# Illumina/canvas

Measured on AMD Instinct MI355X. Metric: genome-bins/sec (bin+clean+partition), higher is better.
Workload: dtype u8/int32 (bin), f32/f64 (clean, viterbi); 1 GPU; BASELINE configs[2]: whole-genome GRCh38 60x single sample, full bin+clean+partition HIP path on 1 MI355X per sample; bins_after_clean=4686240, bin_size=534, partition=PerSampleHMM, clean_flags=-g -s -r --local-sd-metric-file, segments=250, samples=1

## Files before the change

canvas_amd/csrc/hmm.hip:

```cpp
#include "common.hpp"
#include <type_traits>
#include "select.hpp"
#include "quantize.hpp"
#include <mutex>
#include <cmath>
#include <thread>
#include <cstring>
#include <limits>
#include <algorithm>

#define NSTATE 5

struct HmmParams {
    double logA[NSTATE][NSTATE];
    double logPi[NSTATE];
    int32_t tableLen;
    double maxThreshold;
};

__global__ void __launch_bounds__(256) k_keys_cov_f32(const double* __restrict__ cov, int64_t n, uint32_t* __restrict__ keys) {
    int64_t i = (int64_t)blockIdx.x * 256 + threadIdx.x;
    if (i < n) keys[i] = key_of_float((float)cov[i]);
}

// ... 260 lines not shown
struct __attribute__((aligned(2))) VecH8 { uint32_t w[4]; };

template <int J, bool TWO = false>
__device__ __forceinline__ void vit_state(const double (&d)[NSTATE], double e, const HmmParams& P, double& outDelta, uint32_t& outArg) {
    const double NEG = -1.7976931348623157e308;
    const double cOff = e + P.logA[J == 0 ? 1 : 0][J], cDiag = e + P.logA[J][J];
    const double t_0 = d[0] + (TWO ? (J == 0 ? cDiag : cOff) : (e + P.logA[0][J]));
    const double t_1 = d[1] + (TWO ? (J == 1 ? cDiag : cOff) : (e + P.logA[1][J]));
    const double t_2 = d[2] + (TWO ? (J == 2 ? cDiag : cOff) : (e + P.logA[2][J]));
    const double t_3 = d[3] + (TWO ? (J == 3 ? cDiag : cOff) : (e + P.logA[3][J]));
    const double t_4 = d[4] + (TWO ? (J == 4 ? cDiag : cOff) : (e + P.logA[4][J]));
    double a = __builtin_fmax(__builtin_fmax(__builtin_fmax(t_0, t_1), __builtin_fmax(t_2, t_3)), t_4);
    uint32_t ia = t_3 == a ? 3u : 4u;
    ia = t_2 == a ? 2u : ia; ia = t_1 == a ? 1u : ia; ia = t_0 == a ? 0u : ia;
    if (!(a > NEG)) { a = NEG; ia = 0; }
    outDelta = a; outArg = ia;
}
template <bool TWO = false>
__device__ __forceinline__ uint32_t vit_step5(double (&d)[NSTATE], const double (&e)[NSTATE], const HmmParams& P) {
    double n0, n1, n2, n3, n4; uint32_t a0, a1, a2, a3, a4;
    vit_state<0, TWO>(d, e[0], P, n0, a0); vit_state<1, TWO>(d, e[1], P, n1, a1); vit_state<2, TWO>(d, e[2], P, n2, a2);
    vit_state<3, TWO>(d, e[3], P, n3, a3); vit_state<4, TWO>(d, e[4], P, n4, a4);
    d[0] = n0; d[1] = n1; d[2] = n2; d[3] = n3; d[4] = n4;
    return a0 | (a1 << 3) | (a2 << 6) | (a3 << 9) | (a4 << 12);
}
__device__ __forceinline__ void vit_init5(double (&d)[NSTATE], const double (&e)[NSTATE], const HmmParams& P) {
#pragma unroll
    for (int j = 0; j < NSTATE; j++) { double lik = e[j] + P.logA[0][j]; d[j] = P.logPi[j] + lik - P.logA[0][j]; }
}
__device__ __forceinline__ int vit_best5(const double (&d)[NSTATE]) {
    int best = -1; double m1 = -1.7976931348623157e308;
#pragma unroll
    for (int i = 0; i < NSTATE; i++) if (d[i] > m1) { best = i; m1 = d[i]; }
    return best;
}
__device__ __forceinline__ uint32_t map_get(uint32_t m, uint32_t j) { return (m >> (3u * j)) & 7u; }
__device__ __forceinline__ uint32_t map_compose(uint32_t outer, uint32_t inner) {
    return map_get(outer, map_get(inner, 0)) | (map_get(outer, map_get(inner, 1)) << 3) | (map_get(outer, map_get(inner, 2)) << 6) |
           (map_get(outer, map_get(inner, 3)) << 9) | (map_get(outer, map_get(inner, 4)) << 12);
}
__device__ __forceinline__ double sel5(const double (&d)[NSTATE], uint32_t i) {
    double r = d[0];
    r = i == 1 ? d[1] : r; r = i == 2 ? d[2] : r; r = i == 3 ? d[3] : r; r = i == 4 ? d[4] : r;
    return r;
}
__device__ __forceinline__ void vit_emissions(double (&e)[NSTATE], const double* __restrict__ sTab, const double* __restrict__ logPmf, bool useLds, int tableLen, int k) {
    if (useLds) {
#pragma unroll
        for (int j = 0; j < NSTATE; j++) e[j] = sTab[k * NSTATE + j];
    } else {
#pragma unroll
        for (int j = 0; j < NSTATE; j++) e[j] = logPmf[(size_t)j * tableLen + k];
    }
}
__device__ __forceinline__ void vit_stage_table(double* sTab, const double* __restrict__ logPmf, int tableLen, bool useLds) {
    if (useLds) for (int i = threadIdx.x; i < tableLen * NSTATE; i += blockDim.x) { int s = i / tableLen, k = i - s * tableLen; sTab[k * NSTATE + s] = logPmf[i]; }
    __syncthreads();
}
__device__ __forceinline__ int wave_max_i32(int v) {
#pragma unroll
    for (int d = 32; d >= 1; d >>= 1) { int o = __shfl_xor(v, d); v = o > v ? o : v; }
    return v;
}

template <typename T> __device__ __forceinline__ void make_block_entry(const int32_t* __restrict__ first, int nchr, int i, int per, T* __restrict__ out) {
    int lo = 0, hi = nchr - 1;
    while (lo < hi) { int mid = (lo + hi + 1) >> 1; if (first[mid] <= i) lo = mid; else hi = mid - 1; }
    while (lo < nchr - 1 && first[lo + 1] <= i) lo++;
    T b; b.chrom = lo; b.t0 = (i - first[lo]) * per;
    out[i] = b;
}
template <typename T>
__global__ void __launch_bounds__(256) k_make_blocks(const int32_t* __restrict__ first, int nchr, int n, int per, T* __restrict__ out) {
    const int i = blockIdx.x * 256 + threadIdx.x;
    if (i < n) make_block_entry(first, nchr, i, per, out);
}

#define HMM_BYVAL 64
struct HmmDescPack { HmmChrom chroms[HMM_BYVAL]; int64_t off[HMM_BYVAL + 1]; int32_t first[HMM_BYVAL + 1], firstChunk[HMM_BYVAL + 1], firstS[HMM_BYVAL + 1], firstGroup[HMM_BYVAL + 1]; };
struct HmmDescDev { HmmChrom* chroms; int64_t* off; int32_t* first; int32_t* firstChunk; int32_t* firstS; int32_t* firstGroup; };
template <typename VB_T, typename BB_T>
__global__ void __launch_bounds__(256) k_hmm_setup(const HmmDescPack pack, int usePack, HmmDescDev D, int nchr,
                                                   int nblocks, int nblocksS, int nchunks, int vb, int vbs, int bbChunk, VB_T* __restrict__ vBlocks, VB_T* __restrict__ sBlocks, BB_T* __restrict__ bChunks,
                                                   const double* __restrict__ cov, int64_t N, double maxThreshold, int32_t* __restrict__ idx, int32_t* __restrict__ dLast, int32_t* __restrict__ dFail) {
    const int32_t* first = usePack ? pack.first : D.first; const int32_t* firstS = usePack ? pack.firstS : D.firstS; const int32_t* firstChunk = usePack ? pack.firstChunk : D.firstChunk;
    if (usePack && blockIdx.x == 0) {
        for (int c = threadIdx.x; c < nchr; c += 256) D.chroms[c] = pack.chroms[c];
        for (int c = threadIdx.x; c <= nchr; c += 256) { D.off[c] = pack.off[c]; D.first[c] = pack.first[c]; D.firstChunk[c] = pack.firstChunk[c]; D.firstS[c] = pack.firstS[c]; D.firstGroup[c] = pack.firstGroup[c]; }
    }
    const int64_t i = (int64_t)blockIdx.x * 256 + threadIdx.x;
    if (i < nblocks) make_block_entry(first, nchr, (int)i, vb, vBlocks);
    if (i < nblocksS) make_block_entry(firstS, nchr, (int)i, vbs, sBlocks);
    if (i < nchunks) make_block_entry(firstChunk, nchr, (int)i, bbChunk, bChunks);
    if (i < nchr) { dLast[i] = -1; dFail[i] = 0; }
    if (cov && i < N) {
        double x = cov[i];
        x = x > maxThreshold ? maxThreshold : x;
        const int32_t k = (int32_t)rint(x);
        idx[i] = k < 0 ? 0 : k;
    }
}

template <bool useLds, bool TWO>
__global__ void __launch_bounds__(64) k_vit_spec(const VitBlock* __restrict__ blocks, int nblocks, const HmmChrom* __restrict__ chroms, const int32_t* __restrict__ idx,
                                                 const double* __restrict__ logPmf, HmmParams P, uint16_t* __restrict__ psi, uint16_t* __restrict__ maps,
                                                 int32_t* __restrict__ lastGuess, int leadIn, const int32_t* __restrict__ todo, int vb) {
    extern __shared__ double sTab[];
    vit_stage_table(sTab, logPmf, P.tableLen, useLds);
    const int b = blockIdx.x * 64 + threadIdx.x;
    const bool actBlock = b < nblocks;
    const VitBlock B = blocks[actBlock ? b : nblocks - 1];
    const HmmChrom C = chroms[B.chrom];
    const int64_t tBeg = B.t0, tEnd = (B.t0 + vb < C.T) ? B.t0 + vb : C.T;
    const int64_t ts = tBeg > leadIn ? tBeg - leadIn : 0;
    const bool act = actBlock && (!todo || todo[B.chrom]);
    const int nsteps = act ? (int)(tEnd - ts) : 0;
    const int maxSteps = wave_max_i32(nsteps);
    const int32_t* __restrict__ ix = idx + C.begin + ts;
    uint16_t* __restrict__ pp = psi + C.begin;
    double d[NSTATE] = {0.0, 0.0, 0.0, 0.0, 0.0};
    uint32_t fm = MAP_IDENT;
    const int lead = (int)(tBeg - ts);
    if (nsteps > 0) {
        double e[NSTATE];
        vit_emissions(e, sTab, logPmf, useLds, P.tableLen, ix[0]);
        if (ts == 0) vit_init5(d, e, P);
        else {
#pragma unroll
            for (int j = 0; j < NSTATE; j++) d[j] = e[j];
        }
        if (lead == 0) pp[ts] = 0;
    }
    VecI4 qa = *reinterpret_cast<const VecI4*>(ix + 1), qb = *reinterpret_cast<const VecI4*>(ix + 5);
    double eCur[NSTATE];
    vit_emissions(eCur, sTab, logPmf, useLds, P.tableLen, 1 < nsteps ? qa.v[0] : 0);
    auto group = [&](int s0, auto withMaps) {
        constexpr bool WM = decltype(withMaps)::value;
        const VecI4 na = *reinterpret_cast<const VecI4*>(ix + s0 + PQ), nb = *reinterpret_cast<const VecI4*>(ix + s0 + PQ + 4);
        uint32_t pks[PQ];
#pragma unroll
        for (int u = 0; u < PQ; u++) {
            const int s = s0 + u;
            const bool on = s < nsteps;
            const int kNext = (s + 1 < nsteps) ? (u + 1 < 4 ? qa.v[(u + 1) & 3] : (u + 1 < 8 ? qb.v[(u + 1) & 3] : na.v[0])) : 0;
            double eNext[NSTATE], dn[NSTATE];
            vit_emissions(eNext, sTab, logPmf, useLds, P.tableLen, kNext);
#pragma unroll
            for (int j = 0; j < NSTATE; j++) dn[j] = d[j];
            const uint32_t pk = vit_step5<TWO>(dn, eCur, P);
#pragma unroll
            for (int j = 0; j < NSTATE; j++) { d[j] = on ? dn[j] : d[j]; eCur[j] = eNext[j]; }
            if (WM) { fm = (on && s >= lead) ? map_compose(fm, pk) : fm; pks[u] = pk; }
        }
        if (WM) {
#pragma unroll
            for (int u = 0; u < PQ; u++) { const int s = s0 + u; if (s < nsteps && s >= lead) pp[ts + s] = (uint16_t)pks[u]; }
        }
        qa = na; qb = nb;
    };
    const int leadMin = -wave_max_i32(nsteps > 0 ? -lead : -0x7FFFFFFF);
    int s0 = 1;
    for (; s0 + PQ <= leadMin && s0 < maxSteps; s0 += PQ) group(s0, std::false_type{});
    for (; s0 < maxSteps; s0 += PQ) group(s0, std::true_type{});
    if (act) {
        maps[b] = (uint16_t)fm;
        if (tEnd == C.T) lastGuess[B.chrom] = vit_best5(d);
    }
}

#define CHR_LDS_CAP 1024
__device__ __forceinline__ const int64_t* stage_chr_offsets(const int64_t* __restrict__ chrOff, int nchr, int64_t* sOff) {
    if (nchr + 1 > CHR_LDS_CAP) return chrOff;
    for (int k = threadIdx.x; k <= nchr; k += blockDim.x) sOff[k] = chrOff[k];
    __syncthreads();
    return sOff;
}
__device__ __forceinline__ int chrom_of_bin(const int64_t* off, int nchr, int64_t g) {
    int lo = 0, hi = nchr - 1;
    while (lo < hi) { const int mid = (lo + hi + 1) >> 1; if (off[mid] <= g) lo = mid; else hi = mid - 1; }
    return lo;
}
#define VBS (VB / 2)
__global__ void __launch_bounds__(256) k_pair_maps(const VitBlock* __restrict__ blocks, int nblocks, const HmmChrom* __restrict__ chroms, const int32_t* __restrict__ firstS,
                                                   const uint16_t* __restrict__ mapsS, uint16_t* __restrict__ maps, const int32_t* __restrict__ todo) {
    const int b = blockIdx.x * 256 + threadIdx.x;
    if (b >= nblocks) return;
    const VitBlock B = blocks[b];
    if (todo && !todo[B.chrom]) return;
    const int64_t T = chroms[B.chrom].T;
    const int s0 = firstS[B.chrom] + B.t0 / VBS;
    uint32_t m = mapsS[s0];
#pragma unroll
    for (int k = 1; k < VB / VBS; k++) if (B.t0 + (int64_t)k * VBS < T) m = map_compose(m, mapsS[s0 + k]);
    maps[b] = (uint16_t)m;
}

__global__ void __launch_bounds__(256) k_vit_increments(const HmmChrom* __restrict__ chroms, int nchr, const int64_t* __restrict__ chrOff, const int32_t* __restrict__ idx,
                                                        const double* __restrict__ logPmf, HmmParams P, const int32_t* __restrict__ state, int64_t N, double* __restrict__ D) {
    __shared__ int64_t sOff[CHR_LDS_CAP];
    const int64_t* off = stage_chr_offsets(chrOff, nchr, sOff);
    int64_t g = (int64_t)blockIdx.x * 256 + threadIdx.x;
    if (g >= N) return;
    const int s1 = state[g], sPrev = state[g > 0 ? g - 1 : 0], ix = idx[g];
    const int lo = chrom_of_bin(off, nchr, g);
    const int64_t begin = chroms[lo].begin;
    if (s1 < 0) { D[g] = 0.0; return; }
    double e = logPmf[(size_t)s1 * P.tableLen + ix];
    if (g == begin) { double lik = e + P.logA[0][s1]; D[g] = P.logPi[s1] + lik - P.logA[0][s1]; }
    else { const int s0 = sPrev; D[g] = e + P.logA[s0 < 0 ? 0 : s0][s1]; }
}

__global__ void __launch_bounds__(64) k_vit_backbone(const HmmChrom* __restrict__ chroms, const double* __restrict__ V, double* __restrict__ carryOut, const int32_t* __restrict__ todo = nullptr) {
    __shared__ double sV[2][64];
    const HmmChrom C = chroms[blockIdx.x];
    if (C.T <= 10 || (todo && !todo[blockIdx.x])) return;
    const int l = threadIdx.x;
    const double* __restrict__ Vc = V + C.begin;
    double acc = 0.0;
    double vNext = l < C.T ? Vc[l] : 0.0;
    int buf = 0;
    for (int64_t c0 = 0; c0 < C.T; c0 += 64, buf ^= 1) {
        sV[buf][l] = vNext;
        { int64_t t2 = c0 + 64 + l; vNext = t2 < C.T ? Vc[t2] : 0.0; }
        if (l == 0) carryOut[C.begin + c0] = acc;
        double r[64];
#pragma unroll
        for (int s = 0; s < 64; s++) r[s] = sV[buf][s];
#pragma unroll
        for (int s = 0; s < 64; s++) acc = acc + r[s];
    }
}

#define BS_T 1024
#define BS_I 8
struct ParFn { unsigned long long a0, a1; };
__device__ __forceinline__ ParFn parfn_then(ParFn f, ParFn g) {
    ParFn h;
    h.a0 = f.a0 + ((f.a0 & 1ull) ? g.a1 : g.a0);
    h.a1 = f.a1 + ((f.a1 & 1ull) ? g.a0 : g.a1);
    return h;
}
__device__ __forceinline__ ParFn parfn_shfl_up(ParFn f, int d) {
    ParFn o;
    o.a0 = __shfl_up(f.a0, d); o.a1 = __shfl_up(f.a1, d);
    return o;
}
__global__ void __launch_bounds__(BS_T) k_vit_backbone_scan(const HmmChrom* __restrict__ chroms, const double* __restrict__ V, double* __restrict__ carryOut, int32_t* __restrict__ fail) {
    __shared__ ParFn sAgg[BS_T / 64];
    __shared__ long long sCross, sP;
    __shared__ double sM;
    __shared__ int sBad;
    const HmmChrom C = chroms[blockIdx.x];
    if (C.T <= 10) return;
    const int tid = threadIdx.x, lane = tid & 63, wave = tid >> 6;
    const double* __restrict__ Vc = V + C.begin;
    double* __restrict__ carry = carryOut + C.begin;
    const unsigned long long TWO53 = 1ull << 53, MANT = (1ull << 52) - 1ull;
    if (tid == 0) { carry[0] = 0.0; sM = 0.0; sP = 0; sBad = 0; sCross = 0x7fffffffffffffffll; }
    __syncthreads();
    for (;;) {
        const long long p = sP; const double M = sM; const int bad = sBad;
        __syncthreads();
        if (bad || p >= C.T) break;
        if (!(M >= 2.2250738585072014e-308)) {
            if (tid == 0) {
                const double v = Vc[p];
                const unsigned long long vb = (unsigned long long)__double_as_longlong(v);
                if (((vb >> 52) & 0x7ffull) == 0x7ffull || (!(vb >> 63) && (vb << 1) != 0ull)) { sBad = 1; fail[blockIdx.x] = 1; }
                else { const double acc = (0.0 - M) + v; if (((p + 1) & 63) == 0 && p + 1 < C.T) carry[p + 1] = acc; sM = -acc; sP = p + 1; }
            }
            __syncthreads();
            continue;
        }
        const unsigned long long mb = (unsigned long long)__double_as_longlong(M);
        const int eM = (int)((mb >> 52) & 0x7ffull);
        const unsigned long long k0 = (mb & MANT) | (1ull << 52);
        const long long base = p + (long long)tid * BS_I;
        ParFn f[BS_I]; bool myBad = false;
#pragma unroll
        for (int i = 0; i < BS_I; i++) {
            const long long t = base + i;
            unsigned long long A = 0; int r = 0;
            if (t < C.T) {
                const unsigned long long vb = (unsigned long long)__double_as_longlong(Vc[t]);
                const int ea = (int)((vb >> 52) & 0x7ffull);
                if (ea == 0x7ff || (!(vb >> 63) && (vb << 1) != 0ull)) myBad = true;
                const unsigned long long ma = ea ? ((vb & MANT) | (1ull << 52)) : (vb & MANT);
                const int shift = eM - (ea ? ea : 1);
                if (shift <= 0) { if (ma) A = TWO53; }
                else if (shift < 64) {
                    A = ma >> shift;
                    const unsigned long long rem = ma & ((1ull << shift) - 1ull), half = 1ull << (shift - 1);
// ... 118 lines not shown
    const BbChunk K = chunks[blockIdx.x];
    const HmmChrom C = chroms[K.chrom];
    const double* __restrict__ Vc = V + C.begin;
    const int tid = threadIdx.x, lane = tid & 63, wave = tid >> 6;
    unsigned long long vb[4]; double a[4]; bool in[4];
#pragma unroll
    for (int i = 0; i < 4; i++) {
        const int64_t t = (int64_t)K.t0 + tid * 4 + i;
        in[i] = t < C.T;
        const double v = in[i] ? Vc[t] : 0.0;
        vb[i] = (unsigned long long)__double_as_longlong(v); a[i] = fabs(v);
    }
    const double tsum = ((a[0] + a[1]) + a[2]) + a[3];
    double inc = tsum;
#pragma unroll
    for (int d = 1; d < 64; d <<= 1) { double o = shfl_up_f64(inc, d); if (lane >= d) inc += o; }
    if (lane == 63) swSum[wave] = inc;
    __syncthreads();
    double base = chunkBase[blockIdx.x];
    for (int w = 0; w < wave; w++) base += swSum[w];
    double Mprev = base + (inc - tsum);
    SegFn el[4];
#pragma unroll
    for (int i = 0; i < 4; i++) {
        const double Mcur = Mprev + a[i];
        const int ep = (int)(((unsigned long long)__double_as_longlong(Mprev) >> 52) & 0x7ffull), ec = (int)(((unsigned long long)__double_as_longlong(Mcur) >> 52) & 0x7ffull);
        const bool cross = in[i] && (ep == 0 || ec != ep);
        el[i].head = cross ? 1u : 0u; el[i].cnt = cross ? 1u : 0u;
        if (cross || !in[i]) { el[i].f.a0 = 0; el[i].f.a1 = 0; }
        else el[i].f = parfn_of(vb[i], ep);
        a[i] = Mcur;
        Mprev = Mcur;
    }
    SegFn th = el[0];
#pragma unroll
    for (int i = 1; i < 4; i++) th = segfn_then(th, el[i]);
    SegFn sc = th;
#pragma unroll
    for (int d = 1; d < 64; d <<= 1) {
        SegFn o; o.f = parfn_shfl_up(sc.f, d); o.head = __shfl_up(sc.head, d); o.cnt = __shfl_up(sc.cnt, d);
        if (lane >= d) sc = segfn_then(o, sc);
    }
    if (lane == 63) swSeg[wave] = sc;
    __syncthreads();
    SegFn ex; ex.f.a0 = 0; ex.f.a1 = 0; ex.head = 0; ex.cnt = 0;
    for (int w = 0; w < wave; w++) ex = segfn_then(ex, swSeg[w]);
    { SegFn o; o.f = parfn_shfl_up(sc.f, 1); o.head = __shfl_up(sc.head, 1); o.cnt = __shfl_up(sc.cnt, 1); if (lane > 0) ex = segfn_then(ex, o); }
    SegFn run = ex;
    BbCross* __restrict__ myCross = outCross + (size_t)blockIdx.x * BB_MAXC;
    bool overflow = false;
#pragma unroll
    for (int i = 0; i < 4; i++) {
        const int pos = tid * 4 + i;
        if (el[i].head) {
            if (run.cnt < BB_MAXC) {
                BbCross R; R.before = run.f; R.v = __longlong_as_double((long long)vb[i]);
                R.pos = pos; R.e = (int)(((unsigned long long)__double_as_longlong(a[i]) >> 52) & 0x7ffull);
                myCross[run.cnt] = R;
            } else overflow = true;
        }
        run = segfn_then(run, el[i]);
        if ((pos & 63) == 63) {
            at64Fn[(size_t)blockIdx.x * 16 + (pos >> 6)] = run.f;
            at64Rank[(size_t)blockIdx.x * 16 + (pos >> 6)] = (uint8_t)((run.cnt > 127u ? 127u : run.cnt) | (el[i].head ? 0x80u : 0u));
        }
    }
    if (overflow) fail[K.chrom] = 1;
    if (tid == 0) {
        outChunk[blockIdx.x].headE = (int)(((unsigned long long)__double_as_longlong(base) >> 52) & 0x7ffull);
    }
    if (tid == 255) { outChunk[blockIdx.x].tail = run.f; outChunk[blockIdx.x].nCross = (int32_t)run.cnt; }
}
__device__ __forceinline__ bool bb_apply(unsigned long long& bits, const ParFn& f, int eUsed) {
    const unsigned long long MANT = (1ull << 52) - 1ull;
    if (f.a0 == 0ull && f.a1 == 0ull) return true;
    const int e = (int)(bits >> 52);
    if (e != eUsed || e == 0) return false;
    const unsigned long long k = (bits & MANT) | (1ull << 52);
    const unsigned long long k2 = k + ((k & 1ull) ? f.a1 : f.a0);
    if (k2 >= (1ull << 53)) return false;
    bits = ((unsigned long long)e << 52) | (k2 & MANT);
    return true;
}
__global__ void __launch_bounds__(64) k_bb_walk(const int32_t* __restrict__ firstChunk, const BbChunkOut* __restrict__ chunkOut, const BbCross* __restrict__ cross,
                                                unsigned long long* __restrict__ chunkBits, BbPost* __restrict__ post, int32_t* __restrict__ fail) {
    __shared__ BbCross sCr[BB_MAXC];
    const int c = blockIdx.x, l = threadIdx.x;
    const unsigned long long MANT = (1ull << 52) - 1ull;
    if (fail[c]) return;
    unsigned long long bits = 0ull;
    bool failed = false;
    for (int g = firstChunk[c]; g < firstChunk[c + 1] && !failed; g += 64) {
        const int n = firstChunk[c + 1] - g < 64 ? firstChunk[c + 1] - g : 64;
        BbChunkOut my; my.tail.a0 = 0; my.tail.a1 = 0; my.nCross = 0; my.headE = 0;
        if (l < n) my = chunkOut[g + l];
        unsigned long long crossMask = __ballot(l < n && my.nCross > 0);
        int cur = 0;
        while (cur < n && !failed) {
            const int f = crossMask ? (int)__builtin_ctzll(crossMask) : n;
            if (f > cur) {
                const bool inRun = l >= cur && l < f;
                ParFn inc; inc.a0 = inRun ? my.tail.a0 : 0ull; inc.a1 = inRun ? my.tail.a1 : 0ull;
#pragma unroll
                for (int d = 1; d < 64; d <<= 1) { ParFn o = parfn_shfl_up(inc, d); if (l >= d) inc = parfn_then(o, inc); }
                ParFn ex = parfn_shfl_up(inc, 1); if (l == 0) { ex.a0 = 0; ex.a1 = 0; }
                const int e = (int)(bits >> 52);
                const unsigned long long k = (bits & MANT) | (e ? (1ull << 52) : 0ull);
                const unsigned long long ks = k + ((k & 1ull) ? ex.a1 : ex.a0), ke = k + ((k & 1ull) ? inc.a1 : inc.a0);
                const bool nonEmpty = my.tail.a0 != 0ull || my.tail.a1 != 0ull;
                const bool bad = inRun && nonEmpty && (my.headE != e || e == 0 || ke >= (1ull << 53));
                if (inRun) chunkBits[g + l] = ((unsigned long long)e << 52) | (ks & MANT);
                if (__ballot(bad)) failed = true;
                const unsigned long long totLo0 = __shfl(inc.a0, f - 1), totLo1 = __shfl(inc.a1, f - 1);
                const unsigned long long k2 = k + ((k & 1ull) ? totLo1 : totLo0);
                bits = ((unsigned long long)e << 52) | (k2 & MANT);
                cur = f;
            }
            if (cur < n && !failed) {
                const int nc = __shfl(my.nCross, cur), headE = __shfl(my.headE, cur);
                ParFn tail; tail.a0 = __shfl(my.tail.a0, cur); tail.a1 = __shfl(my.tail.a1, cur);
                if (l < nc && l < BB_MAXC) sCr[l] = cross[(size_t)(g + cur) * BB_MAXC + l];
                __builtin_amdgcn_fence(__ATOMIC_ACQ_REL, "wavefront"); __builtin_amdgcn_wave_barrier();
                if (l == 0) chunkBits[g + cur] = bits;
                int eCur = headE;
                for (int r = 0; r < nc && r < BB_MAXC && !failed; r++) {
                    const BbCross R = sCr[r];
                    if (!bb_apply(bits, R.before, eCur)) { failed = true; break; }
                    const double acc = -__longlong_as_double((long long)bits) + R.v;
                    bits = (unsigned long long)__double_as_longlong(-acc) & ~(1ull << 63);
                    if ((int)(bits >> 52) != R.e) failed = true;
                    if (l == 0) post[(size_t)(g + cur) * BB_MAXC + r].bits = bits;
                    eCur = R.e;
                }
                if (!failed && !bb_apply(bits, tail, eCur)) failed = true;
                __builtin_amdgcn_fence(__ATOMIC_ACQ_REL, "wavefront"); __builtin_amdgcn_wave_barrier();
                crossMask &= ~(1ull << cur);
                cur++;
            }
        }
    }
    if (failed && l == 0) fail[c] = 1;
}
__global__ void __launch_bounds__(256) k_bb_emit(const BbChunk* __restrict__ chunks, int nchunks, const HmmChrom* __restrict__ chroms, const unsigned long long* __restrict__ chunkBits,
                                                 const BbPost* __restrict__ post, const ParFn* __restrict__ at64Fn, const uint8_t* __restrict__ at64Rank, double* __restrict__ carryOut) {
    const int i = blockIdx.x * 256 + threadIdx.x;
    const int c = i >> 4, q = i & 15;
    if (c >= nchunks) return;
    const BbChunk K = chunks[c];
    const HmmChrom C = chroms[K.chrom];
    if (q == 0 && K.t0 == 0) carryOut[C.begin] = 0.0;
    const int64_t t = (int64_t)K.t0 + q * 64 + 63;
    if (t + 1 >= C.T) return;
    const unsigned long long MANT = (1ull << 52) - 1ull;
    const uint32_t rk = at64Rank[i];
    const uint32_t rank = (rk & 0x7fu) > (uint32_t)BB_MAXC ? (uint32_t)BB_MAXC : (rk & 0x7fu);
    unsigned long long bits = rank == 0 ? chunkBits[c] : post[(size_t)c * BB_MAXC + (rank - 1)].bits;
    if (!(rk & 0x80u)) {
        const ParFn f = at64Fn[i];
        if (f.a0 != 0ull || f.a1 != 0ull) {
            const unsigned long long k = (bits & MANT) | (1ull << 52);
            const unsigned long long k2 = k + ((k & 1ull) ? f.a1 : f.a0);
            bits = (bits & ~MANT) | (k2 & MANT);
        }
    }
    carryOut[C.begin + t + 1] = -__longlong_as_double((long long)bits);
}

struct LogA25 { double a00, a01, a02, a03, a04, a10, a11, a12, a13, a14, a20, a21, a22, a23, a24, a30, a31, a32, a33, a34, a40, a41, a42, a43, a44; };
// ... 67 lines not shown
            for (int u = 0; u < PQ; u++) { const bool in = j0 + PQ + u < cnt; kn[u] = in ? ixp[j0 + PQ + u] : 0; sn[u] = in ? stp[j0 + PQ + u] : 0; vn[u] = in ? vp[j0 + PQ + u] : 0.0; }
#pragma unroll
            for (int u = 0; u < 4; u++) pn.w[u] = (uint32_t)(j0 + PQ + 2 * u < cnt ? ppp[j0 + PQ + 2 * u] : (uint16_t)0) | ((uint32_t)(j0 + PQ + 2 * u + 1 < cnt ? ppp[j0 + PQ + 2 * u + 1] : (uint16_t)0) << 16);
        }
#pragma unroll
        for (int u = 0; u < PQ; u++) {
            if (LEAD) ver_lead_step<useLds>(S, A, sTab, logPmf, P.tableLen, j0 + u < cnt, kq[u], sq[u], vq[u], pq[u]);
            else ver_block_step<useLds>(S, P, sTab, logPmf, j0 + u < cnt, kq[u], sq[u], vq[u], pq[u]);
        }
        __builtin_amdgcn_sched_barrier(0);
#pragma unroll
        for (int u = 0; u < PQ; u++) { kq[u] = kn[u]; sq[u] = sn[u]; vq[u] = vn[u]; pq[u] = (pn.w[u >> 1] >> (16 * (u & 1))) & 0xFFFFu; }
    }
}
template <bool useLds>
__global__ void __launch_bounds__(64) k_vit_verify(const VitBlock* __restrict__ blocks, int nblocks, const HmmChrom* __restrict__ chroms, const int32_t* __restrict__ idx,
                                                   const double* __restrict__ logPmf, HmmParams P, const uint16_t* __restrict__ psi,
                                                   const int32_t* __restrict__ state, const double* __restrict__ V, const double* __restrict__ carry, const int32_t* __restrict__ lastGuess,
                                                   int32_t* __restrict__ fail, int leadIn, const int32_t* __restrict__ todo) {
    extern __shared__ double sTab[];
    vit_stage_table(sTab, logPmf, P.tableLen, useLds);
    const int b = blockIdx.x * 64 + threadIdx.x;
    const bool actBlock = b < nblocks;
    const VitBlock B = blocks[actBlock ? b : nblocks - 1];
    const HmmChrom C = chroms[B.chrom];
    const int64_t tBeg = B.t0, tEnd = (B.t0 + VB < C.T) ? B.t0 + VB : C.T;
    const int64_t ts = tBeg > leadIn ? tBeg - leadIn : 0;
    const bool act = actBlock && (!todo || todo[B.chrom]);
    const int nsteps = act ? (int)(tEnd - ts) : 0;
    const int maxSteps = wave_max_i32(nsteps);
    const int32_t* __restrict__ ix = idx + C.begin + ts;
    const int32_t* __restrict__ st = state + C.begin + ts;
    const double* __restrict__ Vc = V + C.begin + ts;
    const uint16_t* __restrict__ pp = psi + C.begin + ts;
    VerState S;
#pragma unroll
    for (int j = 0; j < NSTATE; j++) S.d[j] = 0.0;
    S.valid = 0; S.bad = false; S.why = 0;
    S.Dprev = carry[C.begin + ts];
    S.sPrev = ts > 0 ? state[C.begin + ts - 1] : -1;
    LogA25 A;
#define LOGA_LOAD(i, j) A.a##i##j = P.logA[i][j]; asm volatile("" : "+v"(A.a##i##j));
    LOGA_LOAD(0, 0) LOGA_LOAD(0, 1) LOGA_LOAD(0, 2) LOGA_LOAD(0, 3) LOGA_LOAD(0, 4) LOGA_LOAD(1, 0) LOGA_LOAD(1, 1) LOGA_LOAD(1, 2) LOGA_LOAD(1, 3) LOGA_LOAD(1, 4)
    LOGA_LOAD(2, 0) LOGA_LOAD(2, 1) LOGA_LOAD(2, 2) LOGA_LOAD(2, 3) LOGA_LOAD(2, 4) LOGA_LOAD(3, 0) LOGA_LOAD(3, 1) LOGA_LOAD(3, 2) LOGA_LOAD(3, 3) LOGA_LOAD(3, 4)
    LOGA_LOAD(4, 0) LOGA_LOAD(4, 1) LOGA_LOAD(4, 2) LOGA_LOAD(4, 3) LOGA_LOAD(4, 4)
#undef LOGA_LOAD
    const int lead = (int)(tBeg - ts);
    if (nsteps > 0) {
        if (ts == 0) {
            double e[NSTATE];
            vit_emissions(e, sTab, logPmf, useLds, P.tableLen, ix[0]);
            const double Dt = S.Dprev + Vc[0];
            const int sCur = st[0];
            vit_init5(S.d, e, P); S.valid = 31u;
            if (sel5(S.d, (uint32_t)sCur) != Dt) { S.bad = true; S.why |= 16u; }
            S.Dprev = Dt; S.sPrev = sCur;
        } else ver_lead_step<useLds>(S, A, sTab, logPmf, P.tableLen, true, ix[0], st[0], Vc[0], (uint32_t)pp[0]);
    }
    const int start2 = lead > 1 ? lead : 1;
    ver_phase<useLds, true>(S, A, P, sTab, logPmf, ix + 1, st + 1, Vc + 1, pp + 1, nsteps > 0 && lead > 1 ? lead - 1 : 0);
    ver_phase<useLds, false>(S, A, P, sTab, logPmf, ix + start2, st + start2, Vc + start2, pp + start2, nsteps > start2 ? nsteps - start2 : 0);
    double (&d)[NSTATE] = S.d; const uint32_t valid = S.valid; bool bad = S.bad;
    uint32_t why = S.why;
    if (act && tEnd == C.T) { if (valid != 31u || vit_best5(d) != lastGuess[B.chrom]) { bad = true; why |= 32u; } }
    if (act && bad) atomicOr(&fail[B.chrom], (int32_t)(1u | why));
}

__global__ void k_vit_corrupt(uint16_t* __restrict__ psi, int64_t at, int j) {
    if (threadIdx.x == 0 && blockIdx.x == 0) { const uint32_t sh = 3u * (uint32_t)j; uint32_t v = psi[at], p = (v >> sh) & 7u; psi[at] = (uint16_t)((v & ~(7u << sh)) | (((p + 1u) % 5u) << sh)); }
}

__global__ void __launch_bounds__(256) k_bt_maps(const VitBlock* __restrict__ blocks, int nblocks, const HmmChrom* __restrict__ chroms, const uint16_t* __restrict__ psi,
                                                 uint16_t* __restrict__ maps) {
    int b = blockIdx.x * 256 + threadIdx.x;
    if (b >= nblocks) return;
    const VitBlock B = blocks[b];
    const HmmChrom C = chroms[B.chrom];
    const int64_t tBeg = B.t0 > 0 ? B.t0 : 1, tEnd = (B.t0 + VB < C.T) ? B.t0 + VB : C.T;
    uint32_t m = MAP_IDENT;
    for (int64_t t = tEnd - 1; t >= tBeg; t--) m = map_compose(psi[C.begin + t], m);
    maps[b] = (uint16_t)m;
}
__global__ void __launch_bounds__(64) k_bt_group(const int32_t* __restrict__ firstBlock, const int32_t* __restrict__ firstGroup, int nchr, const uint16_t* __restrict__ maps,
                                                 uint16_t* __restrict__ pre, uint16_t* __restrict__ gmap) {
    const int g = blockIdx.x, l = threadIdx.x;
    int lo = 0, hi = nchr - 1;
    while (lo < hi) { const int mid = (lo + hi + 1) >> 1; if (firstGroup[mid] <= g) lo = mid; else hi = mid - 1; }
    while (lo < nchr - 1 && firstGroup[lo + 1] <= g) lo++;
    const int first = firstBlock[lo], last = firstBlock[lo + 1] - 1;
    const int bi = last - ((g - firstGroup[lo]) * 64 + l);
    uint32_t f = bi >= first ? (uint32_t)maps[bi] : MAP_IDENT;
#pragma unroll
    for (int dlt = 1; dlt < 64; dlt <<= 1) { const uint32_t o = __shfl_up(f, dlt); if (l >= dlt) f = map_compose(f, o); }
    const uint32_t ex = __shfl_up(f, 1);
    if (bi >= first) pre[bi] = (uint16_t)(l == 0 ? MAP_IDENT : ex);
    if (l == 63) gmap[g] = (uint16_t)f;
}
__global__ void __launch_bounds__(64) k_bt_gchain(const int32_t* __restrict__ firstGroup, const int32_t* __restrict__ lastState, const uint16_t* __restrict__ gmap,
                                                  int8_t* __restrict__ gentry) {
    const int c = blockIdx.x, l = threadIdx.x;
    const int g0 = firstGroup[c], ng = firstGroup[c + 1] - g0;
    int s = lastState[c];
    for (int base = 0; base < ng; base += 64) {
        uint32_t f = base + l < ng ? (uint32_t)gmap[g0 + base + l] : MAP_IDENT;
#pragma unroll
        for (int dlt = 1; dlt < 64; dlt <<= 1) { const uint32_t o = __shfl_up(f, dlt); if (l >= dlt) f = map_compose(f, o); }
        const uint32_t ex = __shfl_up(f, 1);
        if (base + l < ng) gentry[g0 + base + l] = (int8_t)(s < 0 ? s : (l == 0 ? s : (int)map_get(ex, (uint32_t)s)));
        const uint32_t all = (uint32_t)__builtin_amdgcn_readlane((int)f, 63);
        if (s >= 0) s = (int)map_get(all, (uint32_t)s);
    }
}
__global__ void __launch_bounds__(256) k_bt_states(const VitBlock* __restrict__ blocks, int nblocks, const HmmChrom* __restrict__ chroms, const uint16_t* __restrict__ psi,
                                                   const int32_t* __restrict__ firstBlock, const int32_t* __restrict__ firstGroup, const uint16_t* __restrict__ pre,
                                                   const int8_t* __restrict__ gentry, int32_t* __restrict__ state) {
    static_assert(VB <= 128, "two steps per lane");
    const int b = blockIdx.x * 4 + (threadIdx.x >> 6), l = lane_id();
    if (b >= nblocks) return;
    const VitBlock B = blocks[b];
    const HmmChrom C = chroms[B.chrom];
    const int64_t tBeg = B.t0, tEnd = (B.t0 + VB < C.T) ? B.t0 + VB : C.T;
    const int cnt = (int)(tEnd - tBeg);
    const int sg = gentry[firstGroup[B.chrom] + (firstBlock[B.chrom + 1] - 1 - b) / 64];
    const int s = sg < 0 ? sg : (int)map_get((uint32_t)pre[b], (uint32_t)sg);
    const int j0 = 2 * l, j1 = 2 * l + 1;
    const uint32_t a0 = (j0 >= 1 && j0 < cnt) ? (uint32_t)psi[C.begin + tEnd - j0] : MAP_IDENT;
    const uint32_t a1 = (j1 < cnt) ? (uint32_t)psi[C.begin + tEnd - j1] : MAP_IDENT;
    const uint32_t x1 = map_compose(a1, a0);
    uint32_t v = x1;
#pragma unroll
    for (int d = 1; d < 64; d <<= 1) { const uint32_t o = __shfl_up(v, d); if (l >= d) v = map_compose(v, o); }
    uint32_t ex = __shfl_up(v, 1);
    if (l == 0) ex = MAP_IDENT;
    const uint32_t m0 = map_compose(a0, ex), m1 = map_compose(x1, ex);
    if (j0 < cnt) state[C.begin + tEnd - 1 - j0] = s < 0 ? s : (int)map_get(m0, (uint32_t)s);
    if (j1 < cnt) state[C.begin + tEnd - 1 - j1] = s < 0 ? s : (int)map_get(m1, (uint32_t)s);
}

__global__ void __launch_bounds__(256) k_fill_i32(int32_t* __restrict__ p, int64_t begin, int64_t end, int32_t v) {
    int64_t i = begin + (int64_t)blockIdx.x * 256 + threadIdx.x;
    if (i < end) p[i] = v;
}

__global__ void __launch_bounds__(256) k_seg_flags(const int64_t* __restrict__ chrOff, int nchr, const int32_t* __restrict__ state, const int32_t* __restrict__ start,
                                                   const int32_t* __restrict__ stop, int64_t n, int32_t maxDist, const int64_t* __restrict__ exclOff,
                                                   const int32_t* __restrict__ exclStart, const int32_t* __restrict__ exclStop,
                                                   const int64_t* __restrict__ plOff, const int32_t* __restrict__ plStart, const int32_t* __restrict__ plEnd, const int32_t* __restrict__ plCn,
                                                   uint8_t* __restrict__ flags) {
    __shared__ int64_t sOff[CHR_LDS_CAP];
    const int64_t* off = stage_chr_offsets(chrOff, nchr, sOff);
    int64_t i = (int64_t)blockIdx.x * 256 + threadIdx.x;
    if (i >= n) return;
    const int64_t im = i > 0 ? i - 1 : 0;
    const int32_t st = state[i], stPrev = state[im], stopPrev = stop[im], stopHere = stop[i], startHere = start[i];
    const int lo = chrom_of_bin(off, nchr, i);
    const bool first = (i == off[lo]);
    bool newSeg = st >= 0 && (first || stPrev != st);
    if (exclOff) {
        const uint32_t prevEnd = first ? 0u : (uint32_t)stopPrev;
        int64_t a = exclOff[lo], b = exclOff[lo + 1];
        while (a < b) { int64_t mid = (a + b) >> 1; if ((int64_t)exclStop[mid] < (int64_t)prevEnd) a = mid + 1; else b = mid; }
        if (a < exclOff[lo + 1]) {
            const int forbiddenZoneMid = (exclStart[a] + exclStop[a]) / 2;
            if ((int64_t)prevEnd < forbiddenZoneMid && (int64_t)(uint32_t)stopHere >= forbiddenZoneMid) newSeg = true;
        }
    }
    if (!newSeg && !first) {
        uint32_t prevEnd = (uint32_t)stopPrev;
        if (prevEnd > 0 && maxDist >= 0 && (uint64_t)prevEnd + (uint64_t)maxDist < (uint64_t)(uint32_t)startHere) newSeg = true;
    }
    if (!newSeg && plOff) {
        const uint32_t prevEnd = first ? 0u : (uint32_t)stopPrev;
        const int qs = prevEnd > 0 ? (int)prevEnd : 1, qe = (int)(uint32_t)stopHere;
        int bc0 = 0, bc1 = 0, bc2 = qe - qs + 1, bc3 = 0, bc4 = 0;
        for (int64_t k = plOff[lo]; k < plOff[lo + 1]; k++) {
            const int p = plCn[k];
            if (p == 2) continue;
            const int overlapStart = max(qs - 1, plStart[k] - 1);
            if (overlapStart > plEnd[k]) continue;
            const int overlapBases = min(qe, plEnd[k]) - overlapStart;
            if (overlapBases <= 0) continue;
            bc2 -= overlapBases;
            bc0 += p == 0 ? overlapBases : 0; bc1 += p == 1 ? overlapBases : 0; bc3 += p == 3 ? overlapBases : 0; bc4 += p == 4 ? overlapBases : 0;
        }
        if ((bc0 > 0) + (bc1 > 0) + (bc2 > 0) + (bc3 > 0) + (bc4 > 0) >= 2) newSeg = true;
    }
    flags[i] = newSeg;
}
__global__ void __launch_bounds__(256) k_count_blocks(const uint8_t* __restrict__ flags, int64_t n, uint32_t* __restrict__ blockCnt) {
    __shared__ uint32_t sh[4];
    int64_t base = (int64_t)blockIdx.x * 2048;
    uint32_t c = 0;
    for (int jj = 0; jj < 8; jj++) { int64_t i = base + jj * 256 + threadIdx.x; if (i < n) c += flags[i]; }
    c = wave_reduce_add_u32(c);
    if (lane_id() == 0) sh[threadIdx.x >> 6] = c;
    __syncthreads();
    if (threadIdx.x == 0) blockCnt[blockIdx.x] = sh[0] + sh[1] + sh[2] + sh[3];
}
__global__ void __launch_bounds__(1024) k_scan_blocks2(uint32_t* __restrict__ blockCnt, int nblocks, unsigned long long* __restrict__ total, unsigned* __restrict__ totalSeq = nullptr, unsigned seq = 0) {
    __shared__ uint32_t sh[17];
    uint32_t carry = 0;
    for (int base = 0; base < nblocks; base += 1024) {
        int i = base + threadIdx.x;
        uint32_t v = i < nblocks ? blockCnt[i] : 0;
        uint32_t inc = wave_inclusive_scan_u32(v);
        int w = threadIdx.x >> 6;
        if (lane_id() == 63) sh[w] = inc;
        __syncthreads();
        if (threadIdx.x == 0) { uint32_t s = 0; for (int k = 0; k < 16; k++) { uint32_t t = sh[k]; sh[k] = s; s += t; } sh[16] = s; }
        __syncthreads();
        if (i < nblocks) blockCnt[i] = carry + sh[w] + inc - v;
        carry += sh[16];
        __syncthreads();
    }
    if (threadIdx.x == 0) { *total = carry; if (totalSeq) cvx_mail_publish(totalSeq, seq); }
}
__global__ void __launch_bounds__(256) k_seg_ids(const uint8_t* __restrict__ flags, const uint32_t* __restrict__ blockOff, int64_t n, int32_t* __restrict__ segId) {
    __shared__ uint32_t sh[4];
    int64_t base = (int64_t)blockIdx.x * 2048;
// ... 141 lines not shown
    void finish() {
        for (;;) {
            NbJob j;
            { std::lock_guard<std::mutex> lk(mu); if (next >= jobs.size()) break; j = jobs[next++]; }
            negative_binomial_log_table(j.mean, j.variance, j.len, j.out);
            { std::lock_guard<std::mutex> lk(mu); --pending; }
        }
        std::unique_lock<std::mutex> lk(mu); cvDone.wait(lk, [&] { return pending == 0; });
    }
};

static void quartile_idx(int64_t n, int64_t* idx, int& cnt) {
    cnt = 0;
    int64_t mid = n / 2;
    if (n % 2 == 0) {
        int64_t mm = mid / 2;
        idx[cnt++] = mid - 1; idx[cnt++] = mid;
        if (mid % 2 == 0) { idx[cnt++] = mm - 1; idx[cnt++] = mm; idx[cnt++] = mid + mm - 1; idx[cnt++] = mid + mm; }
        else { idx[cnt++] = mm; idx[cnt++] = mm + mid; }
    } else {
        idx[cnt++] = mid;
        if ((n - 1) % 4 == 0) { int64_t k = (n - 1) / 4; idx[cnt++] = k - 1; idx[cnt++] = k; idx[cnt++] = 3 * k; idx[cnt++] = 3 * k + 1; }
        else { int64_t k = (n - 3) / 4; idx[cnt++] = k; idx[cnt++] = k + 1; idx[cnt++] = 3 * k + 1; idx[cnt++] = 3 * k + 2; }
    }
}
static void quartile_val(int64_t n, const float* v, float& q1, float& q2, float& q3) {
    int64_t mid = n / 2;
    if (n % 2 == 0) {
        q2 = (v[0] + v[1]) / 2;
        if (mid % 2 == 0) { q1 = (v[2] + v[3]) / 2; q3 = (v[4] + v[5]) / 2; } else { q1 = v[2]; q3 = v[3]; }
    } else {
        q2 = v[0];
        if ((n - 1) % 4 == 0) { q1 = (v[1] * 0.25f) + (v[2] * 0.75f); q3 = (v[3] * 0.75f) + (v[4] * 0.25f); }
        else { q1 = (v[1] * 0.75f) + (v[2] * 0.25f); q3 = (v[3] * 0.25f) + (v[4] * 0.75f); }
    }
}

static inline unsigned nblk2(int64_t n, int per) { return (unsigned)((n + per - 1) / per); }

struct HmmLists {
    std::vector<HmmChrom> chroms;
    std::vector<int32_t> firstBlock, firstGroup, firstS, firstChunk;
    int nblocks = 0, ngroups = 0, nblocksS = 0, nchunks = 0;
};
static HmmLists hmm_lists(int32_t nchr, const int64_t* h_chr_offset) {
    HmmLists L;
    L.chroms.resize(nchr); L.firstBlock.resize(nchr + 1);
    for (int c = 0; c < nchr; c++) {
        L.chroms[c].begin = h_chr_offset[c]; L.chroms[c].T = h_chr_offset[c + 1] - h_chr_offset[c];
        L.firstBlock[c] = L.nblocks;
        if (L.chroms[c].T > 10) L.nblocks += (int)((L.chroms[c].T + VB - 1) / VB);
    }
    L.firstBlock[nchr] = L.nblocks;
    L.firstGroup.resize(nchr + 1);
    for (int c = 0; c < nchr; c++) { L.firstGroup[c] = L.ngroups; L.ngroups += (L.firstBlock[c + 1] - L.firstBlock[c] + 63) / 64; }
    L.firstGroup[nchr] = L.ngroups;
    L.firstS.resize(nchr + 1);
    for (int c = 0; c < nchr; c++) { L.firstS[c] = L.nblocksS; if (L.chroms[c].T > 10) L.nblocksS += (int)((L.chroms[c].T + VBS - 1) / VBS); }
    L.firstS[nchr] = L.nblocksS;
    L.firstChunk.resize(nchr + 1);
    for (int c = 0; c < nchr; c++) {
        L.firstChunk[c] = L.nchunks;
        if (L.chroms[c].T > 10) L.nchunks += (int)((L.chroms[c].T + BB_CHUNK - 1) / BB_CHUNK);
    }
    L.firstChunk[nchr] = L.nchunks;
    return L;
}

enum { BB_MODE_CHAIN = 0, BB_MODE_SCAN = 1, BB_MODE_PIECES = 2 };
struct BbWork { double* chunkSum; double* chunkBase; BbChunkOut* chunkOut; BbCross* cross; ParFn* at64Fn; uint8_t* at64Rank; unsigned long long* chunkBits; BbPost* post; };
static void bb_work_size(WsSizer& sz, int nchunks) {
    sz.take<double>(nchunks + 1); sz.take<double>(nchunks + 1); sz.take<BbChunkOut>(nchunks + 1);
    sz.take<BbCross>((size_t)nchunks * BB_MAXC + 1); sz.take<ParFn>((size_t)nchunks * 16 + 1); sz.take<uint8_t>((size_t)nchunks * 16 + 8);
    sz.take<unsigned long long>(nchunks + 1); sz.take<BbPost>((size_t)nchunks * BB_MAXC + 1);
}
static BbWork bb_work_carve(WsCarver& ws, int nchunks) {
    BbWork W;
    W.chunkSum = ws.take<double>(nchunks + 1); W.chunkBase = ws.take<double>(nchunks + 1); W.chunkOut = ws.take<BbChunkOut>(nchunks + 1);
    W.cross = ws.take<BbCross>((size_t)nchunks * BB_MAXC + 1); W.at64Fn = ws.take<ParFn>((size_t)nchunks * 16 + 1); W.at64Rank = ws.take<uint8_t>((size_t)nchunks * 16 + 8);
    W.chunkBits = ws.take<unsigned long long>(nchunks + 1); W.post = ws.take<BbPost>((size_t)nchunks * BB_MAXC + 1);
    return W;
}
static void enqueue_backbone(canvas_ctx* ctx, int mode, int nchr, int nchunks, const HmmChrom* dChroms, const BbChunk* dBChunks, const int32_t* dFirstChunk, const double* dV,
                             double* dCarry, int32_t* dFail, const int32_t* dTodo, const BbWork& W) {
    if (mode == BB_MODE_CHAIN) hipLaunchKernelGGL(k_vit_backbone, dim3(nchr), dim3(64), 0, ctx->stream, dChroms, dV, dCarry, dTodo);
    else if (mode == BB_MODE_SCAN) hipLaunchKernelGGL(k_vit_backbone_scan, dim3(nchr), dim3(BS_T), 0, ctx->stream, dChroms, dV, dCarry, dFail);
    else {
        hipLaunchKernelGGL(k_bb_sums, dim3(nchunks), dim3(256), 0, ctx->stream, dBChunks, dChroms, dV, W.chunkSum, dFail);
        hipLaunchKernelGGL(k_bb_bases, dim3(nchr), dim3(64), 0, ctx->stream, dFirstChunk, W.chunkSum, W.chunkBase);
        hipLaunchKernelGGL(k_bb_pieces, dim3(nchunks), dim3(256), 0, ctx->stream, dBChunks, dChroms, dV, W.chunkBase, W.chunkOut, W.cross, W.at64Fn, W.at64Rank, dFail);
        hipLaunchKernelGGL(k_bb_walk, dim3(nchr), dim3(64), 0, ctx->stream, dFirstChunk, W.chunkOut, W.cross, W.chunkBits, W.post, dFail);
        hipLaunchKernelGGL(k_bb_emit, dim3(nblk2((int64_t)nchunks * 16, 256)), dim3(256), 0, ctx->stream, dBChunks, nchunks, dChroms, W.chunkBits, W.post, W.at64Fn, W.at64Rank, dCarry);
    }
}

struct VitCorrupt { bool on = false, retry = false; int chrom = 0; int64_t t = 0; int state = 2; int attempts = 0; };
static int32_t vit_corrupt_parse(canvas_ctx* ctx, int32_t nchr, const int64_t* h_chr_offset, VitCorrupt& K) {
    const char* s = cvx_hook("CANVAS_HMM_TEST_CORRUPT");
    if (!s) return CANVAS_OK;
    K.on = true;
    if (!strcmp(s, "1")) {
        const int64_t T = h_chr_offset[1] - h_chr_offset[0];
        K.chrom = 0; K.t = T / 2; K.state = 2; K.attempts = T > 10 ? 1 : 0;
        return CANVAS_OK;
    }
    long long v[4] = {0, 0, 0, 0}; int nf = 0; const char* p = s;
    for (;;) {
        char* end = nullptr;
        if (nf == 4 || *p < '0' || *p > '9') { nf = -1; break; }
        v[nf++] = strtoll(p, &end, 10);
        if (end - p > 12) { nf = -1; break; }
        if (*end == 0) break;
        if (*end != ':') { nf = -1; break; }
        p = end + 1;
    }
    if (nf != 3 && nf != 4) CANVAS_FAIL(ctx, CANVAS_ERR_INVALID, "CANVAS_HMM_TEST_CORRUPT: 1, c:t:j or c:t:j:k");
    if (v[0] >= nchr) CANVAS_FAIL(ctx, CANVAS_ERR_INVALID, "CANVAS_HMM_TEST_CORRUPT: no such chromosome");
    const int64_t T = h_chr_offset[v[0] + 1] - h_chr_offset[v[0]];
    if (T <= 10 || v[1] < 1 || v[1] >= T) CANVAS_FAIL(ctx, CANVAS_ERR_INVALID, "CANVAS_HMM_TEST_CORRUPT: the step must be 1 .. T-1 of a chromosome of more than ten bins");
    if (v[2] >= NSTATE) CANVAS_FAIL(ctx, CANVAS_ERR_INVALID, "CANVAS_HMM_TEST_CORRUPT: the state must be 0 .. 4");
    if (nf == 4 && (v[3] < 1 || v[3] > 5)) CANVAS_FAIL(ctx, CANVAS_ERR_INVALID, "CANVAS_HMM_TEST_CORRUPT: 1 .. 5 corrupted attempts");
    K.chrom = (int)v[0]; K.t = v[1]; K.state = (int)v[2]; K.attempts = nf == 4 ? (int)v[3] : 1; K.retry = nf == 4;
    return CANVAS_OK;
}

struct HmmEmis { int32_t* idx = nullptr; double* dTab = nullptr;
                 const double* indexCov = nullptr; };
struct SegPost { const int32_t* d_start; const int32_t* d_stop; int32_t maxDist; int32_t* d_segment_id; int64_t nseg = 0; bool valid = false; };
static void enqueue_segment_ids(canvas_ctx* ctx, const int64_t* dOff, int nchr, const int32_t* d_state, const int32_t* d_start, const int32_t* d_stop, int64_t N, int32_t maxDist,
                                uint8_t* flags, uint32_t* blockCnt, unsigned long long* dTot, int32_t* d_segment_id, unsigned* totSeq = nullptr, unsigned seq = 0);
template <class PrepareA, class PrepareB>
static int32_t hmm_pipeline(canvas_ctx* ctx, int32_t nchr, const int64_t* h_chr_offset, size_t extraBytes, PrepareA prepareA, PrepareB prepareB, int32_t* d_state, SegPost* seg = nullptr,
                            bool descByValue = false ) {
    const int64_t N = h_chr_offset[nchr];
    VitCorrupt corrupt;
    { int32_t rcc = vit_corrupt_parse(ctx, nchr, h_chr_offset, corrupt); if (rcc) return rcc; }
    const HmmLists L = hmm_lists(nchr, h_chr_offset);
    const std::vector<HmmChrom>& chroms = L.chroms;
    const std::vector<int32_t>&firstBlock = L.firstBlock, &firstGroup = L.firstGroup, &firstS = L.firstS, &firstChunk = L.firstChunk;
    const int nblocks = L.nblocks, ngroups = L.ngroups, nblocksS = L.nblocksS, nchunks = L.nchunks;
    const int nbSeg = (int)nblk2(N, 2048);
    WsSizer sz;
    sz.take<BbChunk>(nchunks + 1); sz.take<int32_t>(nchr + 1); bb_work_size(sz, nchunks);
    sz.take<uint16_t>(N + 8); sz.take<HmmChrom>(nchr); sz.take<int32_t>(nchr);
    sz.take<int32_t>(nchr + 1); sz.take<uint16_t>(nblocks + 8); sz.take<int8_t>(nblocks + 8);
    sz.take<int64_t>(nchr + 1); sz.take<VitBlock>(nblocks + 1); sz.take<double>(N); sz.take<double>(N + 64); sz.take<int32_t>(nchr); sz.take<int32_t>(nchr);
    sz.take<VitBlock>(nblocksS + 1); sz.take<uint16_t>(nblocksS + 8); sz.take<int32_t>(nchr + 1);
    sz.take<int32_t>(nchr + 1); sz.take<uint16_t>(nblocks + 8); sz.take<uint16_t>(ngroups + 8); sz.take<int8_t>(ngroups + 8);
    sz.take<char>(8 * 256 + (size_t)nchr * 64 + 64);
    if (seg) { sz.take<uint8_t>(N + 16); sz.take<uint32_t>(nbSeg + 1); sz.take<unsigned long long>(1); }
    int32_t rc = canvas_ws_reserve(ctx, sz.off + extraBytes + 65536); if (rc) return rc;
    rc = canvas_pin_reserve(ctx, (size_t)nchr * 4 + 64); if (rc) return rc;
    WsCarver ws(ctx->ws);
    uint16_t* psi = ws.take<uint16_t>(N + 8);
    HmmChrom* dChroms = ws.take<HmmChrom>(nchr); int32_t* dLast = ws.take<int32_t>(nchr);
    int32_t* dFirst = ws.take<int32_t>(nchr + 1);
    uint16_t* dMaps = ws.take<uint16_t>(nblocks + 8); (void)ws.take<int8_t>(nblocks + 8);
    int64_t* dOffDev = ws.take<int64_t>(nchr + 1);
    VitBlock* dVBlocks = ws.take<VitBlock>(nblocks + 1); double* dD = ws.take<double>(N); double* dCarry = ws.take<double>(N + 64); int32_t* dFail = ws.take<int32_t>(nchr); int32_t* dRedo = ws.take<int32_t>(nchr);
    int32_t* dFirstGroup = ws.take<int32_t>(nchr + 1); uint16_t* dPre = ws.take<uint16_t>(nblocks + 8); uint16_t* dGmap = ws.take<uint16_t>(ngroups + 8);
    int8_t* dGentry = ws.take<int8_t>(ngroups + 8);
    VitBlock* dSBlocks = ws.take<VitBlock>(nblocksS + 1); uint16_t* dMapsS = ws.take<uint16_t>(nblocksS + 8); int32_t* dFirstS = ws.take<int32_t>(nchr + 1);
    BbChunk* dBChunks = ws.take<BbChunk>(nchunks + 1); int32_t* dFirstChunk = ws.take<int32_t>(nchr + 1);
    const BbWork bbWork = bb_work_carve(ws, nchunks);
    uint8_t* segFlags = nullptr; uint32_t* segBlockCnt = nullptr; unsigned long long* segTot = nullptr;
    if (seg) { segFlags = ws.take<uint8_t>(N + 16); segBlockCnt = ws.take<uint32_t>(nbSeg + 1); segTot = ws.take<unsigned long long>(1); seg->valid = false; }

    const bool byVal = descByValue && nchr <= HMM_BYVAL;
    HmmDescPack pack;
    {
        auto al = [](size_t v) { return (v + 255) & ~size_t(255); };
        const size_t oCh = 0, oFirst = al((size_t)nchr * sizeof(HmmChrom)), oOff = oFirst + al((size_t)(nchr + 1) * 4), oChunk = oOff + al((size_t)(nchr + 1) * 8),
                     oS = oChunk + al((size_t)(nchr + 1) * 4), oG = oS + al((size_t)(nchr + 1) * 4), total = oG + al((size_t)(nchr + 1) * 4);
        char* dBlob = ws.take<char>(total);
        if (byVal) {
            memset(&pack, 0, sizeof pack);
            memcpy(pack.chroms, chroms.data(), (size_t)nchr * sizeof(HmmChrom)); memcpy(pack.off, h_chr_offset, (size_t)(nchr + 1) * 8); memcpy(pack.first, firstBlock.data(), (size_t)(nchr + 1) * 4);
            memcpy(pack.firstChunk, firstChunk.data(), (size_t)(nchr + 1) * 4); memcpy(pack.firstS, firstS.data(), (size_t)(nchr + 1) * 4); memcpy(pack.firstGroup, firstGroup.data(), (size_t)(nchr + 1) * 4);
        } else {
            std::vector<char> blob(total, 0);
            memcpy(blob.data() + oCh, chroms.data(), (size_t)nchr * sizeof(HmmChrom)); memcpy(blob.data() + oFirst, firstBlock.data(), (size_t)(nchr + 1) * 4);
            memcpy(blob.data() + oOff, h_chr_offset, (size_t)(nchr + 1) * 8); memcpy(blob.data() + oChunk, firstChunk.data(), (size_t)(nchr + 1) * 4);
            memcpy(blob.data() + oS, firstS.data(), (size_t)(nchr + 1) * 4); memcpy(blob.data() + oG, firstGroup.data(), (size_t)(nchr + 1) * 4);
            rc = canvas_h2d_small(ctx, dBlob, blob.data(), total); if (rc) return rc;
        }
        dChroms = (HmmChrom*)(dBlob + oCh); dFirst = (int32_t*)(dBlob + oFirst); dOffDev = (int64_t*)(dBlob + oOff); dFirstChunk = (int32_t*)(dBlob + oChunk);
        dFirstS = (int32_t*)(dBlob + oS); dFirstGroup = (int32_t*)(dBlob + oG);
    }
    HmmParams P; HmmEmis E;
    ctx->hmm_dispersion = 1e9;
    rc = prepareA(ws, P, E, (const HmmChrom*)dChroms, (const int64_t*)dOffDev); if (rc) return rc;
    {
        const int64_t most = std::max<int64_t>(std::max<int64_t>(E.indexCov ? N : 0, nblocks), std::max<int64_t>(std::max(nblocksS, nchunks), nchr));
        HmmDescDev DD{dChroms, dOffDev, dFirst, dFirstChunk, dFirstS, dFirstGroup};
        hipLaunchKernelGGL((k_hmm_setup<VitBlock, BbChunk>), dim3(nblk2(most, 256)), dim3(256), 0, ctx->stream, pack, byVal ? 1 : 0, DD, nchr, nblocks, nblocksS, nchunks, VB, VBS, BB_CHUNK,
                           dVBlocks, dSBlocks, dBChunks, E.indexCov, N, P.maxThreshold, E.idx, dLast, dFail);
    }
    rc = prepareB(ws, P, E); if (rc) return rc;
    int32_t* idx = E.idx; double* dTab = E.dTab;
    size_t tabBytes = (size_t)NSTATE * P.tableLen * 8;
    size_t lds = tabBytes <= 48 * 1024 ? tabBytes : 0;
    for (int c = 0; c < nchr; c++)
        if (chroms[c].T <= 10 && chroms[c].T > 0)
            hipLaunchKernelGGL(k_fill_i32, dim3(nblk2(chroms[c].T, 256)), dim3(256), 0, ctx->stream, d_state, chroms[c].begin, chroms[c].begin + chroms[c].T, -1);
    const unsigned laneGrid = (unsigned)((nblocks + 63) / 64);
    auto backtrack = [&](bool haveMaps) {
        if (nblocks > 0) {
            if (!haveMaps) hipLaunchKernelGGL(k_bt_maps, dim3(nblk2(nblocks, 256)), dim3(256), 0, ctx->stream, dVBlocks, nblocks, dChroms, psi, dMaps);
            hipLaunchKernelGGL(k_bt_group, dim3(ngroups), dim3(64), 0, ctx->stream, dFirst, dFirstGroup, nchr, dMaps, dPre, dGmap);
            hipLaunchKernelGGL(k_bt_gchain, dim3(nchr), dim3(64), 0, ctx->stream, dFirstGroup, dLast, dGmap, dGentry);
            hipLaunchKernelGGL(k_bt_states, dim3(nblk2(nblocks, 4)), dim3(256), 0, ctx->stream, dVBlocks, nblocks, dChroms, psi, dFirst, dFirstGroup, dPre, dGentry, d_state);
        }
    };
    bool twoValuedAll = true;
    for (int i = 0; i < NSTATE; i++) for (int j = 0; j < NSTATE; j++) {
        const double ref = i == j ? P.logA[0][0] : P.logA[0][1];
        if (memcmp(&P.logA[i][j], &ref, sizeof(double)) != 0) twoValuedAll = false;
    }
    const bool speculative = cvx_hook("CANVAS_HMM_SEQUENTIAL") == nullptr;
    std::vector<int32_t> redo;
    int32_t* hFail = (int32_t*)ctx->pin; unsigned long long* hSegTot = (unsigned long long*)((char*)ctx->pin + (((size_t)nchr * 4 + 15) & ~size_t(15)));
    bool segEnqueued = false; unsigned* hSegSeq = (unsigned*)(hSegTot + 1); unsigned segSeq = 0;
    if (speculative && nblocks > 0) {
        ProfScope ps(ctx, "viterbi");
        const int32_t* dTodo = nullptr;
        ctx->hmm_retry = 0;
        const int vwEnv = cvx_hook("CANVAS_HMM_LEAD") ? atoi(cvx_hook("CANVAS_HMM_LEAD")) : 0;
        const int vw0 = vwEnv > 0 ? vwEnv : (ctx->hmm_dispersion < 0.20 ? VW0 : (ctx->hmm_dispersion < 0.30 ? 64 : VW));
        const int nAttempts = 5;
        for (int attempt = 0; attempt < nAttempts; attempt++) {
            const int mult = attempt <= 1 ? 1 : (attempt == 2 ? 8 : (attempt == 3 ? 64 : 512));
            const int leadSpec = attempt == 0 ? vw0 : mult * VW, leadVer = mult * VW2;
            cvx_prof_count(ctx, "viterbi_attempt");
            if (attempt > 0) CANVAS_HIP_TRY(ctx, hipMemsetAsync(dFail, 0, nchr * 4, ctx->stream));
            const dim3 gs((unsigned)((nblocksS + 63) / 64));
            const bool twoValued = twoValuedAll && attempt < 3;
            if (lds && twoValued) hipLaunchKernelGGL((k_vit_spec<true, true>), gs, dim3(64), lds, ctx->stream, dSBlocks, nblocksS, dChroms, idx, dTab, P, psi, dMapsS, dLast, leadSpec, dTodo, VBS);
            else if (lds) hipLaunchKernelGGL((k_vit_spec<true, false>), gs, dim3(64), lds, ctx->stream, dSBlocks, nblocksS, dChroms, idx, dTab, P, psi, dMapsS, dLast, leadSpec, dTodo, VBS);
            else if (twoValued) hipLaunchKernelGGL((k_vit_spec<false, true>), gs, dim3(64), 0, ctx->stream, dSBlocks, nblocksS, dChroms, idx, dTab, P, psi, dMapsS, dLast, leadSpec, dTodo, VBS);
            else hipLaunchKernelGGL((k_vit_spec<false, false>), gs, dim3(64), 0, ctx->stream, dSBlocks, nblocksS, dChroms, idx, dTab, P, psi, dMapsS, dLast, leadSpec, dTodo, VBS);
            hipLaunchKernelGGL(k_pair_maps, dim3(nblk2(nblocks, 256)), dim3(256), 0, ctx->stream, dVBlocks, nblocks, dChroms, dFirstS, dMapsS, dMaps, dTodo);
            if (attempt < corrupt.attempts) hipLaunchKernelGGL(k_vit_corrupt, dim3(1), dim3(64), 0, ctx->stream, psi, chroms[corrupt.chrom].begin + corrupt.t, corrupt.state);
            backtrack(true);
            hipLaunchKernelGGL(k_vit_increments, dim3(nblk2(N, 256)), dim3(256), 0, ctx->stream, dChroms, nchr, dOffDev, idx, dTab, P, d_state, N, dD);
            const char* bbMode = cvx_hook("CANVAS_HMM_BACKBONE");
            const int bb = ((bbMode && !strcmp(bbMode, "chain")) || (attempt > 1 && !bbMode)) ? BB_MODE_CHAIN : ((bbMode && !strcmp(bbMode, "scan")) ? BB_MODE_SCAN : BB_MODE_PIECES);
            enqueue_backbone(ctx, bb, nchr, nchunks, dChroms, dBChunks, dFirstChunk, dD, dCarry, dFail, dTodo, bbWork);
            if (lds) hipLaunchKernelGGL((k_vit_verify<true>), dim3(laneGrid), dim3(64), lds, ctx->stream, dVBlocks, nblocks, dChroms, idx, dTab, P, psi, d_state, dD, dCarry, dLast, dFail, leadVer, dTodo);
            else hipLaunchKernelGGL((k_vit_verify<false>), dim3(laneGrid), dim3(64), 0, ctx->stream, dVBlocks, nblocks, dChroms, idx, dTab, P, psi, d_state, dD, dCarry, dLast, dFail, leadVer, dTodo);
            CANVAS_HIP_TRY(ctx, hipMemcpyAsync(hFail, dFail, nchr * 4, hipMemcpyDeviceToHost, ctx->stream));
            if (seg && attempt == 0 && (!corrupt.on || corrupt.retry)) {
                (void)segTot;
                segSeq = cvx_mail_arm(ctx, hSegSeq);
                enqueue_segment_ids(ctx, dOffDev, nchr, d_state, seg->d_start, seg->d_stop, N, seg->maxDist, segFlags, segBlockCnt, hSegTot , seg->d_segment_id, hSegSeq, segSeq);
                segEnqueued = true;
            }
            CANVAS_HIP_TRY(ctx, hipStreamSynchronize(ctx->stream));
            redo.clear();
            for (int c = 0; c < nchr; c++) if (hFail[c] && chroms[c].T > 10) redo.push_back(c);
            if (!redo.empty() && cvx_hook("CANVAS_HMM_DEBUG_FAIL")) { fprintf(stderr, "viterbi attempt %d (lead-in x%d):", attempt, mult); for (int c : redo) fprintf(stderr, " chr%d(T=%lld, why=0x%x)", c, (long long)chroms[c].T, (unsigned)hFail[c]); fprintf(stderr, "\n"); }
            if (redo.empty() || (corrupt.on && !corrupt.retry) || cvx_hook("CANVAS_HMM_NO_RETRY")) break;
            if (attempt < nAttempts - 1) {
                if (attempt == 0) { ctx->hmm_retry = (int)redo.size(); { ProfScope pr(ctx, "viterbi_retry"); } }
                int32_t rcq = canvas_h2d_small(ctx, dRedo, hFail, nchr * 4); if (rcq) return rcq;
                dTodo = dRedo;
            }
        }
        if (seg && segEnqueued && redo.empty() && ctx->hmm_retry == 0) { int32_t rcm = cvx_mail_await(ctx, hSegSeq, segSeq, "PerSampleHMM: segment count"); if (rcm) return rcm; seg->valid = true; seg->nseg = (int64_t)*hSegTot; }
    } else {
        for (int c = 0; c < nchr; c++) redo.push_back(c);
    }
    if (!redo.empty()) {
        const bool isFallback = speculative && nblocks > 0;
        ProfScope ps(ctx, isFallback ? "viterbi_sequential" : "viterbi_small");
        if (cvx_hook("CANVAS_HMM_DEBUG_FAIL")) { fprintf(stderr, "viterbi sequential kernel for %zu chromosomes (speculative %d, blocks %d):", redo.size(), (int)speculative, nblocks); for (size_t i = 0; i < redo.size() && i < 6; i++) fprintf(stderr, " chr%d(T=%lld)", redo[i], (long long)chroms[redo[i]].T); fprintf(stderr, "\n"); }
        rc = canvas_h2d_small(ctx, dRedo, redo.data(), redo.size() * 4); if (rc) return rc;
        hipLaunchKernelGGL(k_viterbi, dim3((unsigned)redo.size()), dim3(64), lds, ctx->stream, dChroms, idx, dTab, P, psi, dLast, dRedo);
        backtrack(false);
    }
    ctx->hmm_redo = (int)redo.size();
    CANVAS_HIP_TRY(ctx, hipStreamSynchronize(ctx->stream));
    CANVAS_HIP_TRY(ctx, hipGetLastError());
    return CANVAS_OK;
}

extern "C" {

static int32_t hmm_per_sample_impl(canvas_ctx* ctx, int32_t nchr, const double* d_cov, const int64_t* h_chr_offset, const double* d_cov_all, int64_t nAll, int32_t* d_state, const CovQ* preQ = nullptr, SegPost* seg = nullptr) {
    if (!ctx) return CANVAS_ERR_INVALID;
    if (nchr <= 0 || !d_cov || !h_chr_offset || !d_state || !d_cov_all) CANVAS_FAIL(ctx, CANVAS_ERR_INVALID, "canvas_hmm_per_sample: bad arguments");
    CANVAS_HIP_TRY(ctx, hipSetDevice(ctx->device));
    const int64_t N = h_chr_offset[nchr];
    if (nAll < 5) CANVAS_FAIL(ctx, CANVAS_ERR_UNSUPPORTED, "HMM: fewer than 5 bins genome-wide (Quartiles would throw in the reference)");
    WsSizer ex; ex.take<uint32_t>(nAll); ex.take<int32_t>(N + 256); ex.take<double>(NSTATE * 70000); ex.take<CovQ>(1); ex.take<uint32_t>(CQ_WIN);
    double haploidMean = 0, pseudoVariance = 0;
    std::vector<double> tab;
    struct Joiner { NbPool* p = nullptr; ~Joiner() { if (p) p->finish(); } } joiner;
    auto prepareA = [&](WsCarver& ws, HmmParams& P, HmmEmis& E, const HmmChrom*, const int64_t*) -> int32_t {
        int32_t rc;
        uint32_t* keys = ws.take<uint32_t>(nAll); int32_t* idx = ws.take<int32_t>(N + 256); double* dTab = ws.take<double>(NSTATE * 70000);
    int64_t qidx[6]; int nq;
    quartile_idx(nAll, qidx, nq);
    float v[6], q1, q2, q3;
    bool radix = cvx_hook("CANVAS_HMM_RADIX_SELECT") != nullptr;
    if (!radix && preQ) { rc = cvx_mail_await(ctx, &preQ->pad, ctx->covq_seq, "PerSampleHMM: coverage quartiles"); if (rc) return rc; }
    if (!radix && preQ && preQ->nq == (uint32_t)nq && preQ->n == nAll) {
        bool same = true; for (int k = 0; k < nq; k++) same = same && preQ->rank[k] == (unsigned long long)qidx[k];
        if (same && !preQ->bad && !preQ->fail) for (int k = 0; k < nq; k++) v[k] = (float)((double)preQ->resultK[k] / 100.0);
        else radix = true;
    } else if (!radix) {
        CovQ* dQ = ws.take<CovQ>(1); uint32_t* dWin = ws.take<uint32_t>(CQ_WIN);
        CovQ hQ; memset(&hQ, 0, sizeof hQ); hQ.nq = (uint32_t)nq;
        for (int k = 0; k < nq; k++) hQ.rank[k] = (unsigned long long)qidx[k];
        rc = canvas_h2d_small(ctx, dQ, &hQ, sizeof hQ); if (rc) return rc;
        CANVAS_HIP_TRY(ctx, hipMemsetAsync(dWin, 0, CQ_WIN * 4, ctx->stream));
        hipLaunchKernelGGL(k_covq_hist, dim3(256), dim3(1024), 0, ctx->stream, d_cov_all, nAll, dQ, dWin);
        hipLaunchKernelGGL(k_covq_pick, dim3(1), dim3(1024), 0, ctx->stream, dQ, dWin);
        rc = canvas_pin_reserve(ctx, sizeof(CovQ)); if (rc) return rc;
        CANVAS_HIP_TRY(ctx, hipMemcpyAsync(ctx->pin, dQ, sizeof(CovQ), hipMemcpyDeviceToHost, ctx->stream));
        CANVAS_HIP_TRY(ctx, hipStreamSynchronize(ctx->stream));
        CANVAS_HIP_TRY(ctx, hipGetLastError());
        const CovQ& R = *(const CovQ*)ctx->pin;
        if (R.bad || R.fail) radix = true;
        else for (int k = 0; k < nq; k++) v[k] = (float)((double)R.resultK[k] / 100.0);
    }
    if (radix) {
        hipLaunchKernelGGL(k_keys_cov_f32, dim3(nblk2(nAll, 256)), dim3(256), 0, ctx->stream, d_cov_all, nAll, keys);
        std::vector<SelQuery> qs;
        for (int k = 0; k < nq; k++) qs.push_back({0, 0, qidx[k]});
        std::vector<unsigned long long> res;
        rc = radix_select<uint32_t>(ctx, keys, 1, std::vector<int64_t>{0, nAll}, qs, res); if (rc) return rc;
        for (int k = 0; k < nq; k++) v[k] = host_float_of_key((uint32_t)res[k]);
    }
    quartile_val(nAll, v, q1, q2, q3);
    const double median = (double)q2;
    const float iqr = q3 - q1;
    ctx->hmm_dispersion = q2 > 0 ? (double)iqr / (double)q2 : 1e9;
    pseudoVariance = (double)(iqr * iqr);
    haploidMean = median / 2.0;
    P.maxThreshold = haploidMean * NSTATE;
    if (!(P.maxThreshold >= 0) || P.maxThreshold > 60000) CANVAS_FAIL(ctx, CANVAS_ERR_UNSUPPORTED, "HMM: coverage scale outside the supported table size");
    P.tableLen = (int32_t)std::nearbyint(P.maxThreshold) + 10 + 1;
        E.idx = idx; E.dTab = dTab; E.indexCov = d_cov;
        if (!ctx->hmm_pool) ctx->hmm_pool = std::make_shared<NbPool>(NSTATE - 1);
        (void)lgamma1_table(P.tableLen);
        tab.assign((size_t)NSTATE * P.tableLen, 0.0);
        NbJob jobs[NSTATE];
        for (int CN = 0; CN < NSTATE; CN++) jobs[CN] = NbJob{std::max((double)CN, 0.1) * haploidMean, pseudoVariance, P.tableLen, &tab[(size_t)CN * P.tableLen]};
        joiner.p = static_cast<NbPool*>(ctx->hmm_pool.get());
        joiner.p->submit(jobs, NSTATE);
        return CANVAS_OK;
    };
    auto prepareB = [&](WsCarver&, HmmParams& P, HmmEmis& E) -> int32_t {
    std::static_pointer_cast<NbPool>(ctx->hmm_pool)->finish();
    const double selfTransition = 0.99;
    for (int i = 0; i < NSTATE; i++) {
        for (int j = 0; j < NSTATE; j++) P.logA[i][j] = std::log(i == j ? selfTransition : (1.0 - selfTransition) / (NSTATE - 1));
        P.logPi[i] = std::log((double)(1.0f / NSTATE));
    }
        return canvas_h2d_small(ctx, E.dTab, tab.data(), tab.size() * 8);
    };
// ... 117 lines not shown
        double mx = 0;
        for (int d = 0; d < S; d++) {
            haploid[c * S + d] = std::max(1.0, hMed[c * S + d]) / 2.0;
            variance[c * S + d] = hS2[c * S + d] / (double)(chroms[c].T - 1);
            mx = d == 0 ? haploid[c * S + d] : std::max(mx, haploid[c * S + d]);
        }
        thr[c] = mx * NSTATE;
        if (!(thr[c] >= 0) || thr[c] > 60000) CANVAS_FAIL(ctx, CANVAS_ERR_UNSUPPORTED, "HMM: coverage scale outside the supported table size");
        strideUb = std::max(strideUb, (int)std::nearbyint(thr[c]) + 11);
    }
    JointCombos K; genotype_combinations(S, K);
    WsSizer ex; ex.take<int32_t>(N + 256); ex.take<int32_t>((size_t)S * N); ex.take<double>((size_t)NSTATE * N); ex.take<double>(nCS * NSTATE * strideUb); ex.take<double>(nchr); ex.take<int32_t>(nchr);
    auto prepare = [&](WsCarver& ws, HmmParams& P, HmmEmis& E, const HmmChrom* dChroms, const int64_t* dOffDev) -> int32_t {
        int32_t* idx = ws.take<int32_t>(N + 256); int32_t* idxS = ws.take<int32_t>((size_t)S * N); double* dL = ws.take<double>((size_t)NSTATE * N);
        double* dPmf = ws.take<double>(nCS * NSTATE * strideUb); double* dThr = ws.take<double>(nchr); int32_t* dMaxIdx = ws.take<int32_t>(nchr);
        int32_t rc = canvas_h2d_small(ctx, dThr, thr.data(), nchr * 8); if (rc) return rc;
        CANVAS_HIP_TRY(ctx, hipMemsetAsync(dMaxIdx, 0, nchr * 4, ctx->stream));
        hipLaunchKernelGGL(k_joint_index, dim3(nblk2(N, 256)), dim3(256), 0, ctx->stream, ptrs, S, dOffDev, nchr, dThr, N, idxS, dMaxIdx);
        std::vector<int32_t> hMax(nchr);
        CANVAS_HIP_TRY(ctx, hipMemcpyAsync(hMax.data(), dMaxIdx, nchr * 4, hipMemcpyDeviceToHost, ctx->stream));
        CANVAS_HIP_TRY(ctx, hipStreamSynchronize(ctx->stream));
        int stride = 16;
        for (int c = 0; c < nchr; c++) if (chroms[c].T > 10) stride = std::max(stride, hMax[c] + 10);
        if (stride > strideUb) CANVAS_FAIL(ctx, CANVAS_ERR_HIP, "canvas_hmm_joint: internal table bound exceeded");
        std::vector<double> tab(nCS * NSTATE * (size_t)stride, 0.0);
        parallel_for((int64_t)nCS * NSTATE, 1, [&](int64_t a, int64_t b) {
            for (int64_t i = a; i < b; i++) {
                const int c = (int)(i / (S * NSTATE)), d = (int)((i / NSTATE) % S), CN = (int)(i % NSTATE);
                if (chroms[c].T <= 10) continue;
                negative_binomial_table(std::max((double)CN, 0.1) * haploid[c * S + d], variance[c * S + d], hMax[c] + 10, &tab[(size_t)i * stride]);
            }
        });
        CANVAS_HIP_TRY(ctx, hipMemcpyAsync(dPmf, tab.data(), tab.size() * 8, hipMemcpyHostToDevice, ctx->stream));
        hipLaunchKernelGGL(k_joint_emission, dim3(nblk2(N, 256)), dim3(256), 0, ctx->stream, idxS, S, dOffDev, nchr, dChroms, dPmf, stride, K, N, dL);
        std::vector<double> hL((size_t)NSTATE * N);
        CANVAS_HIP_TRY(ctx, hipMemcpyAsync(hL.data(), dL, hL.size() * 8, hipMemcpyDeviceToHost, ctx->stream));
        CANVAS_HIP_TRY(ctx, hipStreamSynchronize(ctx->stream));
        CANVAS_HIP_TRY(ctx, hipGetLastError());
        parallel_for((int64_t)hL.size(), 1 << 16, [&](int64_t a, int64_t b) { for (int64_t i = a; i < b; i++) hL[i] = std::log(hL[i]); });
        CANVAS_HIP_TRY(ctx, hipMemcpyAsync(dL, hL.data(), hL.size() * 8, hipMemcpyHostToDevice, ctx->stream));
        hipLaunchKernelGGL(k_iota_i32, dim3(nblk2(N, 256)), dim3(256), 0, ctx->stream, idx, N);
        CANVAS_HIP_TRY(ctx, hipStreamSynchronize(ctx->stream));
        P.tableLen = (int32_t)N; P.maxThreshold = 0.0;
        const double selfTransition = 0.99;
        for (int i = 0; i < NSTATE; i++) {
            for (int j = 0; j < NSTATE; j++) P.logA[i][j] = std::log(i == j ? selfTransition : (1.0 - selfTransition) / (NSTATE - 1));
            P.logPi[i] = std::log((double)(1.0f / NSTATE));
        }
        E.idx = idx; E.dTab = dL;
        return CANVAS_OK;
    };
    return hmm_pipeline(ctx, nchr, h_chr_offset, ex.off, prepare, [](WsCarver&, HmmParams&, HmmEmis&) -> int32_t { return CANVAS_OK; }, d_state);
}

extern "C" int32_t canvas_hmm_backbone_probe(canvas_ctx* ctx, int32_t mode, int32_t nchr, const int64_t* h_chr_offset, const double* d_V, double* d_carry, int32_t* h_fail) {
    if (!ctx) return CANVAS_ERR_INVALID;
    if (mode < BB_MODE_CHAIN || mode > BB_MODE_PIECES || nchr < 1 || nchr > (1 << 20) || !h_chr_offset || !h_fail)
        CANVAS_FAIL(ctx, CANVAS_ERR_INVALID, "canvas_hmm_backbone_probe: bad arguments (mode 0..2, 1..2^20 chromosomes)");
    if (h_chr_offset[0] != 0) CANVAS_FAIL(ctx, CANVAS_ERR_INVALID, "canvas_hmm_backbone_probe: the offsets start at 0");
    for (int c = 0; c < nchr; c++) if (h_chr_offset[c + 1] < h_chr_offset[c] || h_chr_offset[c + 1] > (1ll << 30)) CANVAS_FAIL(ctx, CANVAS_ERR_INVALID, "canvas_hmm_backbone_probe: the offsets decrease or pass 2^30 steps");
    const int64_t N = h_chr_offset[nchr];
    if (N > 0 && (!d_V || !d_carry)) CANVAS_FAIL(ctx, CANVAS_ERR_INVALID, "canvas_hmm_backbone_probe: no increments / no room for the carries");
    for (int c = 0; c < nchr; c++) h_fail[c] = 0;
    const HmmLists L = hmm_lists(nchr, h_chr_offset);
    const int nchunks = L.nchunks;
    if (nchunks == 0) return CANVAS_OK;
    CANVAS_HIP_TRY(ctx, hipSetDevice(ctx->device));
    WsSizer sz; sz.take<HmmChrom>(nchr); sz.take<int32_t>(nchr + 1); sz.take<BbChunk>(nchunks + 1); sz.take<int32_t>(nchr); bb_work_size(sz, nchunks);
    int32_t rc = canvas_ws_reserve(ctx, sz.off + 65536); if (rc) return rc;
    WsCarver ws(ctx->ws);
    HmmChrom* dChroms = ws.take<HmmChrom>(nchr); int32_t* dFirstChunk = ws.take<int32_t>(nchr + 1); BbChunk* dBChunks = ws.take<BbChunk>(nchunks + 1); int32_t* dFail = ws.take<int32_t>(nchr);
    const BbWork W = bb_work_carve(ws, nchunks);
    rc = canvas_h2d_small(ctx, dChroms, L.chroms.data(), (size_t)nchr * sizeof(HmmChrom)); if (rc) return rc;
    rc = canvas_h2d_small(ctx, dFirstChunk, L.firstChunk.data(), (size_t)(nchr + 1) * 4); if (rc) return rc;
    CANVAS_HIP_TRY(ctx, hipMemsetAsync(dFail, 0, (size_t)nchr * 4, ctx->stream));
    hipLaunchKernelGGL((k_make_blocks<BbChunk>), dim3(nblk2(nchunks, 256)), dim3(256), 0, ctx->stream, dFirstChunk, nchr, nchunks, BB_CHUNK, dBChunks);
    enqueue_backbone(ctx, mode, nchr, nchunks, dChroms, dBChunks, dFirstChunk, d_V, d_carry, dFail, nullptr, W);
    CANVAS_HIP_TRY(ctx, hipGetLastError());
    CANVAS_HIP_TRY(ctx, hipStreamSynchronize(ctx->stream));
    CANVAS_HIP_TRY(ctx, hipMemcpy(h_fail, dFail, (size_t)nchr * 4, hipMemcpyDeviceToHost));
    return CANVAS_OK;
}

static void enqueue_segment_ids(canvas_ctx* ctx, const int64_t* dOff, int nchr, const int32_t* d_state, const int32_t* d_start, const int32_t* d_stop, int64_t N, int32_t maxDist,
                                uint8_t* flags, uint32_t* blockCnt, unsigned long long* dTot, int32_t* d_segment_id, unsigned* totSeq, unsigned seq) {
    const int nb = (int)nblk2(N, 2048);
    hipLaunchKernelGGL(k_seg_flags, dim3(nblk2(N, 256)), dim3(256), 0, ctx->stream, dOff, nchr, d_state, d_start, d_stop, N, maxDist, (const int64_t*)nullptr, (const int32_t*)nullptr, (const int32_t*)nullptr,
                       (const int64_t*)nullptr, (const int32_t*)nullptr, (const int32_t*)nullptr, (const int32_t*)nullptr, flags);
    hipLaunchKernelGGL(k_count_blocks, dim3(nb), dim3(256), 0, ctx->stream, flags, N, blockCnt);
    hipLaunchKernelGGL(k_scan_blocks2, dim3(1), dim3(1024), 0, ctx->stream, blockCnt, nb, dTot, totSeq, seq);
    hipLaunchKernelGGL(k_seg_ids, dim3(nb), dim3(256), 0, ctx->stream, flags, blockCnt, N, d_segment_id);
}
extern "C" {
int32_t canvas_segment_ids_ploidy(canvas_ctx* ctx, int32_t nchr, const int64_t* h_chr_offset, const int32_t* d_state, const int32_t* d_start,
                                  const int32_t* d_stop, int32_t max_inter_bin_dist, const int64_t* h_excl_offset, const int32_t* h_excl_start,
                                  const int32_t* h_excl_stop, const int64_t* h_ploidy_offset, const int32_t* h_ploidy_start, const int32_t* h_ploidy_end,
                                  const int32_t* h_ploidy_cn, int32_t* d_segment_id, int64_t* h_nsegments) {
    if (!ctx) return CANVAS_ERR_INVALID;
    if (nchr <= 0 || !h_chr_offset || !d_state || !d_start || !d_stop || !d_segment_id) CANVAS_FAIL(ctx, CANVAS_ERR_INVALID, "canvas_segment_ids: bad arguments");
    CANVAS_HIP_TRY(ctx, hipSetDevice(ctx->device));
    const int64_t N = h_chr_offset[nchr];
    if (N == 0) { if (h_nsegments) *h_nsegments = 0; return CANVAS_OK; }
    const int nb = (int)nblk2(N, 2048);
    const int64_t nex = h_excl_offset ? h_excl_offset[nchr] : 0;
    if (h_excl_offset && nex > 0 && (!h_excl_start || !h_excl_stop)) CANVAS_FAIL(ctx, CANVAS_ERR_INVALID, "canvas_segment_ids_filtered: missing interval arrays");
    if (h_excl_offset) for (int c = 0; c < nchr; c++) for (int64_t k = h_excl_offset[c] + 1; k < h_excl_offset[c + 1]; k++)
        if (h_excl_stop[k] < h_excl_stop[k - 1]) CANVAS_FAIL(ctx, CANVAS_ERR_UNSUPPORTED, "forbidden intervals must be sorted by end within a chromosome");
    const int64_t npl = h_ploidy_offset ? h_ploidy_offset[nchr] : 0;
    if (h_ploidy_offset && npl > 0 && (!h_ploidy_start || !h_ploidy_end || !h_ploidy_cn)) CANVAS_FAIL(ctx, CANVAS_ERR_INVALID, "canvas_segment_ids_ploidy: missing ploidy arrays");
    for (int64_t k = 0; k < npl; k++) if (h_ploidy_cn[k] < 0 || h_ploidy_cn[k] > 4)
        CANVAS_FAIL(ctx, CANVAS_ERR_INVALID, "reference ploidy outside 0..4 (PloidyInfo.getPloidyCounts indexes a 5-element array: the reference throws)");
    WsSizer sz; sz.take<int64_t>(nchr + 1); sz.take<uint8_t>(N); sz.take<uint32_t>(nb + 1); sz.take<unsigned long long>(1);
    sz.take<int64_t>(nchr + 1); sz.take<int32_t>(nex + 1); sz.take<int32_t>(nex + 1);
    sz.take<int64_t>(nchr + 1); sz.take<int32_t>(npl + 1); sz.take<int32_t>(npl + 1); sz.take<int32_t>(npl + 1);
    int32_t rc = canvas_ws_reserve(ctx, sz.off + 4096); if (rc) return rc;
    WsCarver ws(ctx->ws);
    int64_t* dOff = ws.take<int64_t>(nchr + 1); uint8_t* flags = ws.take<uint8_t>(N); uint32_t* blockCnt = ws.take<uint32_t>(nb + 1); unsigned long long* dTot = ws.take<unsigned long long>(1);
    int64_t* dExOff = ws.take<int64_t>(nchr + 1); int32_t* dExStart = ws.take<int32_t>(nex + 1); int32_t* dExStop = ws.take<int32_t>(nex + 1);
    int64_t* dPlOff = ws.take<int64_t>(nchr + 1); int32_t* dPlStart = ws.take<int32_t>(npl + 1); int32_t* dPlEnd = ws.take<int32_t>(npl + 1); int32_t* dPlCn = ws.take<int32_t>(npl + 1);
    if (h_ploidy_offset) {
        CANVAS_HIP_TRY(ctx, hipMemcpyAsync(dPlOff, h_ploidy_offset, (nchr + 1) * 8, hipMemcpyHostToDevice, ctx->stream));
        if (npl > 0) { CANVAS_HIP_TRY(ctx, hipMemcpyAsync(dPlStart, h_ploidy_start, npl * 4, hipMemcpyHostToDevice, ctx->stream));
                       CANVAS_HIP_TRY(ctx, hipMemcpyAsync(dPlEnd, h_ploidy_end, npl * 4, hipMemcpyHostToDevice, ctx->stream));
                       CANVAS_HIP_TRY(ctx, hipMemcpyAsync(dPlCn, h_ploidy_cn, npl * 4, hipMemcpyHostToDevice, ctx->stream)); }
    }
    if (h_excl_offset) {
        CANVAS_HIP_TRY(ctx, hipMemcpyAsync(dExOff, h_excl_offset, (nchr + 1) * 8, hipMemcpyHostToDevice, ctx->stream));
        if (nex > 0) { CANVAS_HIP_TRY(ctx, hipMemcpyAsync(dExStart, h_excl_start, nex * 4, hipMemcpyHostToDevice, ctx->stream));
                       CANVAS_HIP_TRY(ctx, hipMemcpyAsync(dExStop, h_excl_stop, nex * 4, hipMemcpyHostToDevice, ctx->stream)); }
    }
    CANVAS_HIP_TRY(ctx, hipMemcpyAsync(dOff, h_chr_offset, (nchr + 1) * 8, hipMemcpyHostToDevice, ctx->stream));
    hipLaunchKernelGGL(k_seg_flags, dim3(nblk2(N, 256)), dim3(256), 0, ctx->stream, dOff, nchr, d_state, d_start, d_stop, N, max_inter_bin_dist, h_excl_offset ? dExOff : (const int64_t*)nullptr, dExStart, dExStop,
                       h_ploidy_offset ? dPlOff : (const int64_t*)nullptr, dPlStart, dPlEnd, dPlCn, flags);
    hipLaunchKernelGGL(k_count_blocks, dim3(nb), dim3(256), 0, ctx->stream, flags, N, blockCnt);
    hipLaunchKernelGGL(k_scan_blocks2, dim3(1), dim3(1024), 0, ctx->stream, blockCnt, nb, dTot);
    hipLaunchKernelGGL(k_seg_ids, dim3(nb), dim3(256), 0, ctx->stream, flags, blockCnt, N, d_segment_id);
    unsigned long long tot = 0;
    CANVAS_HIP_TRY(ctx, hipMemcpyAsync(&tot, dTot, 8, hipMemcpyDeviceToHost, ctx->stream));
    CANVAS_HIP_TRY(ctx, hipStreamSynchronize(ctx->stream));
    CANVAS_HIP_TRY(ctx, hipGetLastError());
    if (h_nsegments) *h_nsegments = (int64_t)tot;
    return CANVAS_OK;
}

int32_t canvas_segment_ids_filtered(canvas_ctx* ctx, int32_t nchr, const int64_t* h_chr_offset, const int32_t* d_state, const int32_t* d_start,
                                    const int32_t* d_stop, int32_t max_inter_bin_dist, const int64_t* h_excl_offset, const int32_t* h_excl_start,
                                    const int32_t* h_excl_stop, int32_t* d_segment_id, int64_t* h_nsegments) {
    return canvas_segment_ids_ploidy(ctx, nchr, h_chr_offset, d_state, d_start, d_stop, max_inter_bin_dist, h_excl_offset, h_excl_start, h_excl_stop,
                                     nullptr, nullptr, nullptr, nullptr, d_segment_id, h_nsegments);
}

int32_t canvas_segment_ids(canvas_ctx* ctx, int32_t nchr, const int64_t* h_chr_offset, const int32_t* d_state, const int32_t* d_start,
                           const int32_t* d_stop, int32_t max_inter_bin_dist, int32_t* d_segment_id, int64_t* h_nsegments) {
    return canvas_segment_ids_filtered(ctx, nchr, h_chr_offset, d_state, d_start, d_stop, max_inter_bin_dist, nullptr, nullptr, nullptr, d_segment_id, h_nsegments);
}

int32_t canvas_split_overlapping(int32_t nsamples, const uint32_t* const* h_start, const uint32_t* const* h_end, const int32_t* h_nseg,
                                 uint32_t* h_out_start, uint32_t* h_out_end, int32_t cap, int32_t* h_nout) {
    if (nsamples <= 0 || !h_start || !h_end || !h_nseg || !h_nout) return CANVAS_ERR_INVALID;
    if (nsamples == 1) {
        if (h_nseg[0] > cap) return CANVAS_ERR_CAPACITY;
        for (int i = 0; i < h_nseg[0]; i++) { h_out_start[i] = h_start[0][i]; h_out_end[i] = h_end[0][i]; }
        *h_nout = h_nseg[0];
        return CANVAS_OK;
    }
    std::vector<std::pair<uint32_t, int>> ev;
    for (int s = 0; s < nsamples; s++) for (int i = 0; i < h_nseg[s]; i++) { ev.push_back({h_start[s][i], 0}); ev.push_back({h_end[s][i], 1}); }
    std::stable_sort(ev.begin(), ev.end(), [](const std::pair<uint32_t, int>& a, const std::pair<uint32_t, int>& b) { return a.first < b.first; });
    int overlapping = 0, n = 0; uint32_t cur = 0;
    for (auto& e : ev) {
        if (overlapping > 0 && cur != e.first) { if (n < cap) { h_out_start[n] = cur; h_out_end[n] = e.first; } n++; }
        cur = e.first; overlapping += e.second == 0 ? 1 : -1;
    }
    *h_nout = n;
    return n > cap ? CANVAS_ERR_CAPACITY : CANVAS_OK;
// ... 4 lines not shown
```

canvas_amd/lib.py:

```python
import sys
import ctypes as C
import os

import numpy as np

HERE = os.path.dirname(os.path.abspath(__file__))
_SO = os.path.join(HERE, "libcanvas_hip.so")
_SYNTH_SO = os.path.join(HERE, "libcanvas_synth.so")

MODE_BINARY, MODE_TDR, MODE_GCW = 0, 3, 5
SELECT_MEDIAN_F32, SELECT_MEDIAN_F64, SELECT_UPPER = 0, 1, 2
LOGISTIC_GERMLINE = (-5.0123, 4.9801, -5.5472, -1.7914)
FILTER_Q10, FILTER_L10KB = 1, 2
CLEAN_GCNORM, CLEAN_FILTSIZE, CLEAN_OUTLIERS, CLEAN_LOCALSD, CLEAN_LOESS = 1, 2, 4, 8, 16

ABI_SYMBOLS = [
    "canvas_create", "canvas_destroy", "canvas_last_error", "canvas_version", "canvas_set_stream", "canvas_set_one_shot", "canvas_synchronize",
    "canvas_device_malloc", "canvas_device_free", "canvas_memcpy_h2d", "canvas_memcpy_d2h", "canvas_host_register", "canvas_host_unregister", "canvas_upload_genome_begin", "canvas_upload_genome_wait",
    "canvas_packed_plane_bytes", "canvas_pack_reference_host", "canvas_pack_hits_host", "canvas_pack_genome_device", "canvas_upload_packed_begin", "canvas_bin_sample_packed", "canvas_sample_pipeline_packed", "canvas_pack_hits2_host", "canvas_upload_packed2_begin",
    "canvas_mask_from_fasta", "canvas_mask_exclude_intervals", "canvas_screen_hits",
    "canvas_bin_rates", "canvas_bin_size_from_rates", "canvas_bin_count_upper_bound", "canvas_bin_genome", "canvas_bin_sample", "canvas_bin_sample_gcweighted", "canvas_bin_predefined", "canvas_bin_predefined_gcweighted",
    "canvas_clean", "canvas_clean2", "canvas_clean_batch", "canvas_merge_cleaned", "canvas_chromosome_offsets", "canvas_quantize_f2", "canvas_hmm_per_sample", "canvas_hmm_joint", "canvas_segment_ids", "canvas_segment_ids_filtered", "canvas_segment_ids_ploidy", "canvas_evenness_score", "canvas_split_overlapping", "canvas_cbs", "canvas_cbs_undo", "canvas_cbs_device_stats", "canvas_cbs_tailp_stats", "canvas_cbs_tail_probe", "canvas_cbs_boundary", "canvas_cbs_seeds", "canvas_cbs_prefetch", "canvas_cbs_stream_read", "canvas_cbs_cache_stats", "canvas_wavelets", "canvas_wavelets_stats", "canvas_wavelets_decisions", "canvas_wavelets_inputs", "canvas_wavelets_prefix_probe", "canvas_wavelets_bound_probe", "canvas_wavelets_level_probe", "canvas_wavelets_chain_probe", "canvas_wavelets_subtree_probe", "canvas_wavelets_median_probe", "canvas_normalize_reference", "canvas_normalize_ratio", "canvas_normalize_best_normal", "canvas_normalize_pca_reference", "canvas_sample_pipeline",
    "canvas_comm_unique_id", "canvas_comm_init", "canvas_comm_init_host", "canvas_allgather_boundaries", "canvas_sample_pipeline_sharded", "canvas_sample_pipeline_sharded_packed", "canvas_sharded_stats", "canvas_cbs_sharded", "canvas_wavelets_sharded", "canvas_allgather_host", "canvas_merge_cleaned_sharded", "canvas_profile_enable", "canvas_profile_get", "canvas_bin_gcw_stats", "canvas_cbs_tpermp_stats", "canvas_comm_split", "canvas_comm_restore", "canvas_comm_rank", "canvas_bin_sample_sharded", "canvas_hmm_per_sample_sharded", "canvas_cbs_perm_probe", "canvas_cbs_arc_probe", "canvas_stale_reads", "canvas_select_probe", "canvas_hmm_backbone_probe",
    "canvas_memcpy_h2d_async", "canvas_snv_count", "canvas_flag_unique_kmers", "canvas_fasta_case_from_mask",
    "canvas_smooth", "canvas_smooth_lengths", "canvas_smooth_plan",
    "canvas_segment_select", "canvas_segment_select_plan", "canvas_call_diploid",
    "canvas_somatic_model_fit", "canvas_call_somatic",
]


SOMATIC_TILE, SOMATIC_MAX_CN = 256, 10
ERR_SOMATIC_NO_MODEL, ERR_SOMATIC_NO_SCORE = -6, -7
SOMATIC_INFO_CLUSTER_TERM, SOMATIC_INFO_INDEX_CUTOFF = 1, 2
SOMATIC_MODEL_VALID, SOMATIC_MODEL_SCORED = 1, 2
SOMATIC_DEFAULTS = dict(maximum_copy_number=8, deviation_index_cutoff=11, maximum_related_models=5, min_allowed_ploidy=0.5, max_allowed_ploidy=8.0, deviation_factor=1.75,
                        cn2_weighting_factor=0.175, deviation_score_weighting_factor=0.375, diploid_distance_score_weighting_factor=0.125,
                        heterogeneity_score_weighting_factor=0.202)


class SomaticParams(C.Structure):
    _fields_ = [("maximum_copy_number", C.c_int32), ("deviation_index_cutoff", C.c_int32), ("maximum_related_models", C.c_int32),
                ("min_allowed_ploidy", C.c_float), ("max_allowed_ploidy", C.c_float), ("deviation_factor", C.c_float),
                ("cn2_weighting_factor", C.c_double), ("deviation_score_weighting_factor", C.c_double), ("diploid_distance_score_weighting_factor", C.c_double),
                ("heterogeneity_score_weighting_factor", C.c_double)]


class SomaticGrid(C.Structure):
    _fields_ = [("min_coverage", C.c_int32), ("max_coverage", C.c_int32), ("minimum_purity_hard_limit", C.c_int32), ("fixed_percent_purity", C.c_int32),
                ("fixed_coverage", C.c_int32), ("is_enrichment", C.c_int32), ("min_minor_allele_coverage", C.c_double), ("coverage_weighting_factor", C.c_double),
                ("genome_length", C.c_int64)]


class SomaticResult(C.Structure):
    _fields_ = [("best_model", C.c_int32), ("best_coverage", C.c_int32), ("best_percent_purity", C.c_int32), ("info", C.c_uint32),
                ("nmodels", C.c_int32), ("nvalid", C.c_int32), ("nscored", C.c_int32), ("reserved", C.c_int32),
                ("diploid_coverage", C.c_double), ("purity", C.c_double), ("deviation", C.c_double), ("precision_deviation", C.c_double), ("accuracy_deviation", C.c_double),
                ("ploidy", C.c_double), ("percent_normal", C.c_double), ("diploid_distance", C.c_double), ("percent_cn", C.c_double * (SOMATIC_MAX_CN + 1)),
                ("score", C.c_double), ("inter_model_distance", C.c_double), ("best_deviation", C.c_double), ("worst_allowed_deviation", C.c_double),
                ("host_table_ms", C.c_double), ("upload_ms", C.c_double), ("device_ms", C.c_double), ("selection_ms", C.c_double)]


class SomaticModels(C.Structure):
    _fields_ = [("capacity", C.c_int64), ("coverage", C.c_void_p), ("percent_purity", C.c_void_p), ("deviation", C.c_void_p), ("precision_deviation", C.c_void_p),
                ("accuracy_deviation", C.c_void_p), ("ploidy", C.c_void_p), ("percent_normal", C.c_void_p), ("percent_cn", C.c_void_p), ("diploid_distance", C.c_void_p),
                ("flags", C.c_void_p), ("score", C.c_void_p)]


ERR_SOMATIC_FEW_SEGMENTS = -8
SOMATIC_MEAN_NONE, SOMATIC_MEAN_WALK, SOMATIC_MEAN_EXACT = -1, 0, 1
SOMATIC_CALL_DEFAULTS = dict(minimum_variant_frequencies=50, minimum_call_size=50000, quality_filter_threshold=10, merge_span=1, is_enrichment=0, minimum_purity_hard_limit=20,
                             lower_coverage_level_weighting_factor=4.0, upper_coverage_level_weighting_factor=2.355, user_purity=-1.0, user_ploidy=-1.0,
                             coverage_weighting=0.333, coverage_weighting_with_maf_segmentation=0.20, evenness_score_threshold=94.5, min_evenness_score=88.0,
                             logistic_intercept=-0.5143, logistic_log_bin_count=0.8596, logistic_model_distance=-50.4366, logistic_distance_ratio=-0.6511,
                             evenness_score=float("nan"), snv_purity_estimate=float("nan"), min_minor_allele_coverage=0.0, genome_length=0)


class SomaticCallParams(C.Structure):
    _fields_ = [("fit", SomaticParams), ("minimum_variant_frequencies", C.c_int32), ("minimum_call_size", C.c_int32), ("quality_filter_threshold", C.c_int32),
                ("merge_span", C.c_int32), ("is_enrichment", C.c_int32), ("minimum_purity_hard_limit", C.c_int32),
                ("lower_coverage_level_weighting_factor", C.c_float), ("upper_coverage_level_weighting_factor", C.c_float), ("user_purity", C.c_float), ("user_ploidy", C.c_float),
                ("coverage_weighting", C.c_double), ("coverage_weighting_with_maf_segmentation", C.c_double), ("evenness_score_threshold", C.c_double),
                ("min_evenness_score", C.c_double), ("logistic_intercept", C.c_double), ("logistic_log_bin_count", C.c_double), ("logistic_model_distance", C.c_double),
                ("logistic_distance_ratio", C.c_double), ("evenness_score", C.c_double), ("snv_purity_estimate", C.c_double), ("min_minor_allele_coverage", C.c_double),
                ("genome_length", C.c_int64)]


SOMATIC_CALL_OUT = [("seg_median_count", np.float64, "seg"), ("seg_site_offset", np.int64, "seg1"), ("seg_maf_upper", np.float64, "seg"), ("seg_usable", np.int32, "seg"),
                    ("seg_coverage", np.float64, "seg"), ("seg_maf", np.float64, "seg"), ("seg_weight", np.float64, "seg"), ("seg_cn", np.int32, "seg"), ("seg_cn2", np.int32, "seg"),
                    ("seg_mcc", np.int32, "seg"), ("seg_dist", np.float64, "seg"), ("seg_dist2", np.float64, "seg"), ("seg_mean_count", np.float64, "seg"),
                    ("seg_mean_route", np.int32, "seg"), ("seg_qscore", np.int32, "seg"), ("seg_run", np.int64, "seg"), ("run_owner", np.int64, "run"), ("run_begin", np.int32, "run"),
                    ("run_end", np.int32, "run"), ("run_bin_count", np.int64, "run"), ("run_qscore", np.int32, "run"), ("run_filter", np.int32, "run")]


class SomaticCallOut(C.Structure):
    _fields_ = [(name, C.c_void_p) for name, _, _ in SOMATIC_CALL_OUT]


class SomaticCallScalars(C.Structure):
    _fields_ = [("nruns", C.c_int64), ("nusable", C.c_int64), ("kept_sites", C.c_int64), ("stages", C.c_int32), ("threshold_used", C.c_int32),
                ("median_coverage_level", C.c_int32), ("min_coverage", C.c_int32), ("max_coverage", C.c_int32), ("fixed_percent_purity", C.c_int32),
                ("overall_median_coverage", C.c_float), ("deviation_factor", C.c_float), ("mean_coverage", C.c_double), ("coverage_weighting_factor", C.c_double),
                ("reported_purity", C.c_double), ("purity_model_fit", C.c_double), ("inter_model_distance", C.c_double), ("estimated_chromosome_count", C.c_double),
                ("heterogeneity_proportion", C.c_double), ("stage1_ms", C.c_double), ("stage23_ms", C.c_double), ("stage4_ms", C.c_double), ("stage5_ms", C.c_double),
                ("stage6_ms", C.c_double)]


# ... 382 lines not shown
        return ms.value, k.value

    def hmm_per_sample(self, cov, chr_offset, out=None):
        torch = self.torch
        off = np.ascontiguousarray(chr_offset, np.int64)
        state = out[:int(off[-1])] if out is not None else torch.empty(int(off[-1]), dtype=torch.int32, device=self.device)
        self._check(self.lib.canvas_hmm_per_sample(self.ctx, len(off) - 1, C.c_void_p(cov.data_ptr()), _np_ptr(off), C.c_void_p(state.data_ptr())))
        return state

    def cbs_device_stats(self):
        out = np.zeros(6, np.int64)
        self._check(self.lib.canvas_cbs_device_stats(self.ctx, _np_ptr(out)))
        return out

    def cbs_tail_probe(self, xs, tol=1e-6):
        xs = np.ascontiguousarray(xs, np.float64); nu = np.zeros(len(xs), np.float64); fl = np.zeros(len(xs), np.int32)
        self._check(self.lib.canvas_cbs_tail_probe(self.ctx, _np_ptr(xs), len(xs), C.c_double(tol), _np_ptr(nu), _np_ptr(fl)))
        return nu, fl

    def cbs_cache_stats(self):
        out = np.zeros(6, np.int64)
        self._check(self.lib.canvas_cbs_cache_stats(self.ctx, _np_ptr(out)))
        return out

    def cbs_stream_read(self, chromosome, position, nwords):
        out = np.zeros(int(nwords), np.uint32)
        self._check(self.lib.canvas_cbs_stream_read(self.ctx, int(chromosome), C.c_int64(int(position)), C.c_int64(int(nwords)), _np_ptr(out)))
        return out

    def cbs_prefetch(self, nchr, words_per_chromosome=0):
        self._check(self.lib.canvas_cbs_prefetch(self.ctx, int(nchr), C.c_int64(int(words_per_chromosome))))

    def cbs_perm_probe(self, x, seed, nb, kernel, tss):
        x = np.ascontiguousarray(x, np.float64)
        lohi = np.zeros((nb, 2), np.float64); ms = np.zeros(3, np.float64)
        self._check(self.lib.canvas_cbs_perm_probe(self.ctx, _np_ptr(x), C.c_int32(len(x)), C.c_uint32(seed & 0xFFFFFFFF), C.c_int32(nb), C.c_int32(kernel), C.c_double(tss), _np_ptr(lohi), _np_ptr(ms)))
        return lohi, ms

    def cbs_arc_probe(self, segments, al0=2, mode=0, pair_cap=0):
        segs = [np.ascontiguousarray(s, np.float64).ravel() for s in segments]
        off = np.zeros(len(segs) + 1, np.int64); off[1:] = np.cumsum([len(s) for s in segs])
        x = np.ascontiguousarray(np.concatenate(segs)) if segs else np.zeros(0, np.float64)
        ns, tot = len(segs), max(1, len(x))
        out = dict(off=off, sx=np.zeros(tot, np.float64), tau=np.zeros(ns, np.float64), stat=np.zeros(ns, np.float64), iseg=np.zeros((ns, 2), np.int32), path=np.zeros(ns, np.int32),
                   words=np.zeros((ns, 6), np.uint64), dmax=np.zeros(tot, np.float64), first=np.zeros(tot, np.int32))
        self._check(self.lib.canvas_cbs_arc_probe(self.ctx, C.c_int32(mode), C.c_int32(ns), _np_ptr(off), _np_ptr(x), C.c_int32(al0), C.c_int32(pair_cap), _np_ptr(out["sx"]), _np_ptr(out["tau"]),
                                                  _np_ptr(out["stat"]), _np_ptr(out["iseg"]), _np_ptr(out["path"]), _np_ptr(out["words"]), _np_ptr(out["dmax"]), _np_ptr(out["first"])))
        return out

    def select_probe(self, variant, dtype, values, seg_off, seg_lo, seg_hi, k):
        want = (np.float32, np.float64, np.uint32, np.uint64)[dtype]
        values = np.ascontiguousarray(values)
        if values.dtype != want:
            raise CanvasError(f"select_probe: dtype {dtype} takes {np.dtype(want).name} values, not {values.dtype.name}")
        off = np.ascontiguousarray(seg_off, np.int64); lo = np.ascontiguousarray(seg_lo, np.int32); hi = np.ascontiguousarray(seg_hi, np.int32)
        kk = np.ascontiguousarray(k, np.int64)
        nq = len(lo)
        if len(hi) != nq or kk.shape != ((nq, 2) if variant == 2 else (nq,)):
            raise CanvasError("select_probe: one (seg_lo, seg_hi, k) per query; k is a pair per query with variant 2")
        if len(off) < 2 or off.max() > len(values):
            raise CanvasError("select_probe: the segment offsets reach past the values")
        bits = values.view(np.int32 if values.itemsize == 4 else np.int64)
        dev = self.torch.from_numpy(bits if len(bits) else np.zeros(1, bits.dtype)).to(self.device)
        out = np.zeros(kk.shape, np.uint64)
        self._check(self.lib.canvas_select_probe(self.ctx, C.c_int32(variant), C.c_int32(dtype), C.c_void_p(dev.data_ptr()), C.c_int32(len(off) - 1), _np_ptr(off), C.c_int32(nq),
                                                 _np_ptr(lo), _np_ptr(hi), _np_ptr(kk), _np_ptr(out)))
        return out

    def backbone_probe(self, mode, v, chr_offset):
        v = np.ascontiguousarray(v)
        if v.dtype != np.float64:
            raise CanvasError(f"backbone_probe: float64 increments, not {v.dtype.name}")
        off = np.ascontiguousarray(chr_offset, np.int64)
        if len(off) < 2 or off[0] != 0 or off[-1] != len(v) or (np.diff(off) < 0).any():
            raise CanvasError("backbone_probe: the offsets start at 0, do not decrease and end at len(v)")
        torch = self.torch
        n = len(v)
        dv = torch.from_numpy(v.view(np.int64) if n else np.zeros(1, np.int64)).to(self.device)
        dc = torch.full((max(n, 1),), BACKBONE_PROBE_UNTOUCHED, dtype=torch.int64, device=self.device)
        torch.cuda.synchronize(self.device)
        fail = np.zeros(len(off) - 1, np.int32)
        self._check(self.lib.canvas_hmm_backbone_probe(self.ctx, C.c_int32(mode), C.c_int32(len(off) - 1), _np_ptr(off), C.c_void_p(dv.data_ptr()), C.c_void_p(dc.data_ptr()), _np_ptr(fail)))
        return dc.cpu().numpy()[:n].view(np.float64), fail

    def stale_reads(self):
        out = np.zeros(2, np.int64)
        self._check(self.lib.canvas_stale_reads(_np_ptr(out)))
        return out

    def cbs_tpermp_stats(self):
        out = np.zeros(2, np.int64)
        self._check(self.lib.canvas_cbs_tpermp_stats(self.ctx, _np_ptr(out)))
        return out

    def cbs_tailp_stats(self):
        out = np.zeros(2, np.int64)
        self._check(self.lib.canvas_cbs_tailp_stats(self.ctx, _np_ptr(out)))
        return out

    def hmm_joint(self, covs, chr_offset, out=None):
        torch = self.torch
        off = np.ascontiguousarray(chr_offset, np.int64)
        state = out[:int(off[-1])] if out is not None else torch.empty(int(off[-1]), dtype=torch.int32, device=self.device)
        ptrs = (C.c_void_p * len(covs))(*[C.c_void_p(c.data_ptr()) for c in covs])
        self._check(self.lib.canvas_hmm_joint(self.ctx, len(covs), len(off) - 1, ptrs, _np_ptr(off), C.c_void_p(state.data_ptr())))
        return state

    def evenness_score(self, cov, chr_offset, window=100000):
        off = np.ascontiguousarray(chr_offset, np.int64)
        score = C.c_double(0); valid = C.c_int32(0)
        self._check(self.lib.canvas_evenness_score(self.ctx, len(off) - 1, C.c_void_p(cov.data_ptr()), _np_ptr(off), int(window), C.byref(score), C.byref(valid)))
        return score.value if valid.value else None

    def snv_count(self, records, offsets, ref_id, site_pos, site_ref, site_alt, ref_counts=None, alt_counts=None, min_mapq=0, min_base_q=20, nbytes=None, want_info=True):
        torch = self.torch
        ns = int(site_pos.numel())
        if ref_counts is None:
            ref_counts = torch.zeros(max(ns, 1), dtype=torch.int32, device=self.device)
        if alt_counts is None:
            alt_counts = torch.zeros(max(ns, 1), dtype=torch.int32, device=self.device)
        assert records.dtype == torch.uint8 and offsets.dtype == torch.int64 and site_pos.dtype == torch.int32 and site_ref.dtype == torch.uint8 and site_alt.dtype == torch.uint8
        assert ref_counts.dtype == torch.int32 and alt_counts.dtype == torch.int32 and ref_counts.numel() >= ns and alt_counts.numel() >= ns
        for t in (records, offsets, site_pos, site_ref, site_alt, ref_counts, alt_counts):
            assert t.is_contiguous() and t.dim() == 1 and (t.numel() == 0 or t.device == self.device), "snv_count: tensors must be dense, one-dimensional and on the context's device"
        nb = int(records.numel()) if nbytes is None else int(nbytes)
        assert 0 <= nb <= records.numel()
        info = np.zeros(5, np.int64) if want_info else None
        self._check(self.lib.canvas_snv_count(self.ctx, C.c_void_p(records.data_ptr()), C.c_uint64(nb), C.c_void_p(offsets.data_ptr()), C.c_int64(int(offsets.numel())),
                                              int(ref_id), int(min_mapq), int(min_base_q), C.c_void_p(site_pos.data_ptr()), C.c_void_p(site_ref.data_ptr()),
                                              C.c_void_p(site_alt.data_ptr()), ns, C.c_void_p(ref_counts.data_ptr()), C.c_void_p(alt_counts.data_ptr()),
                                              _np_ptr(info) if want_info else None))
        return ref_counts, alt_counts, info

    def flag_unique_kmers(self, bases, lens, masks=None, max_table_bytes=0):
        torch = self.torch
        n = len(bases)
        hl = np.ascontiguousarray(lens, np.int64)
        assert len(hl) == n
        if masks is None:
            masks = [torch.empty((int(L) + 63) // 64, dtype=torch.int64, device=self.device) for L in hl]
        for t, m, L in zip(bases, masks, hl):
            assert t.dtype == torch.uint8 and t.is_contiguous() and t.numel() >= L and (L == 0 or t.device == self.device), "flag_unique_kmers: bases must be dense uint8 tensors on the context's device"
            assert m.dtype == torch.int64 and m.is_contiguous() and m.numel() >= (int(L) + 63) // 64 and (L == 0 or m.device == self.device), "flag_unique_kmers: masks must be dense int64 tensors on the context's device"
        st = np.zeros(8, np.int64)
        torch.cuda.synchronize(self.device)
        self._check(self.lib.canvas_flag_unique_kmers(self.ctx, n, _ptr_table(bases), _np_ptr(hl), _ptr_table(masks), C.c_int64(int(max_table_bytes)), _np_ptr(st)))
        return masks, dict(positions=int(st[0]), keyed=int(st[1]), unique=int(st[2]), passes=int(st[3]), table_slots=int(st[4]), longest_probe=int(st[5]), table_bytes=int(st[6]))

    def fasta_case_from_mask(self, bases, length, mask):
        torch = self.torch
        assert bases.dtype == torch.uint8 and bases.is_contiguous() and bases.numel() >= length and mask.dtype == torch.int64 and mask.numel() >= (int(length) + 63) // 64
        torch.cuda.synchronize(self.device)
        self._check(self.lib.canvas_fasta_case_from_mask(self.ctx, C.c_void_p(bases.data_ptr()), C.c_int64(int(length)), C.c_void_p(mask.data_ptr())))
        self.synchronize()
        return bases

    def smooth(self, counts, chr_offset, max_half_window, out=None):
        torch = self.torch
        off = np.ascontiguousarray(chr_offset, np.int64)
        assert off.ndim == 1 and len(off) >= 1
        assert counts.dtype == torch.float32 and counts.is_contiguous() and counts.dim() == 1 and (counts.numel() == 0 or counts.device == self.device), "smooth: counts must be a dense float32 tensor on the context's device"
        assert int(off[-1]) <= counts.numel(), "smooth: the offsets reach past the counts"
        if out is None:
            out = torch.empty_like(counts)
        assert out.dtype == torch.float32 and out.is_contiguous() and out.dim() == 1 and out.numel() >= int(off[-1]) and (out.numel() == 0 or out.device == self.device)
        out_n = np.zeros(max(len(off) - 1, 1), np.int64)
# ... 538 lines not shown
```

include/canvas_hip.h:

```cpp
#ifndef CANVAS_HIP_H
#define CANVAS_HIP_H
#include <stdint.h>
#ifdef __cplusplus
extern "C" {
#endif

typedef struct canvas_ctx canvas_ctx;

enum {
    CANVAS_OK = 0,
    CANVAS_ERR_INVALID = -1,
    CANVAS_ERR_HIP = -2,
    CANVAS_ERR_UNSUPPORTED = -3,
    CANVAS_ERR_CAPACITY = -4,
    CANVAS_ERR_COMM = -5
};

enum { CANVAS_MODE_BINARY = 0, CANVAS_MODE_TRUNCATED_DYNAMIC_RANGE = 3, CANVAS_MODE_GC_CONTENT_WEIGHTED = 5 };

enum { CANVAS_CLEAN_GCNORM = 1, CANVAS_CLEAN_FILTSIZE = 2, CANVAS_CLEAN_OUTLIERS = 4, CANVAS_CLEAN_LOCALSD = 8, CANVAS_CLEAN_LOESS = 16 };

canvas_ctx* canvas_create(int device);
void canvas_destroy(canvas_ctx* ctx);
const char* canvas_last_error(canvas_ctx* ctx);
// ... 32 lines not shown

int32_t canvas_mask_from_fasta(canvas_ctx* ctx, const uint8_t* d_bases, int64_t len, uint64_t* d_mask);
int32_t canvas_mask_exclude_intervals(canvas_ctx* ctx, uint64_t* d_mask, int64_t len, int32_t n, const int32_t* h_start, const int32_t* h_stop);
int32_t canvas_screen_hits(canvas_ctx* ctx, uint8_t* d_hits, const uint64_t* d_mask, int64_t len);
int32_t canvas_bin_rates(canvas_ctx* ctx, int32_t nchr, const uint8_t* const* d_hits, const uint64_t* const* d_mask,
                         const int64_t* h_len, int64_t* h_observed, int64_t* h_possible, double* h_rate);
int32_t canvas_bin_size_from_rates(const double* h_rates, int32_t n, int32_t counts_per_bin);
int64_t canvas_bin_count_upper_bound(int32_t nchr, const int64_t* h_len, int32_t bin_size);
int32_t canvas_bin_genome(canvas_ctx* ctx, int32_t nchr, const uint8_t* const* d_bases, const uint64_t* const* d_mask,
                          const uint8_t* const* d_hits, const int64_t* h_len, int32_t bin_size, int32_t mode,
                          int32_t* d_chr, int32_t* d_start, int32_t* d_stop, int32_t* d_gc, float* d_count, int64_t cap,
                          int64_t* h_nbins_per_chr, int64_t* h_nbins_total);

int32_t canvas_bin_sample(canvas_ctx* ctx, int32_t nchr, const uint8_t* const* d_bases, const uint64_t* const* d_mask,
                          const uint8_t* const* d_hits, const int64_t* h_len, const uint8_t* h_chr_is_autosome,
                          int32_t counts_per_bin, int32_t bin_size_in, int32_t mode,
                          int32_t* d_chr, int32_t* d_start, int32_t* d_stop, int32_t* d_gc, float* d_count, int64_t cap,
                          int32_t* h_bin_size_out, int64_t* h_nbins_per_chr, int64_t* h_nbins_total);

int32_t canvas_bin_sample_gcweighted(canvas_ctx* ctx, int32_t nchr, const uint8_t* const* d_bases, const uint64_t* const* d_mask,
                                     const uint8_t* const* d_hits, const int16_t* const* d_fraglen, const int64_t* h_len,
                                     const uint8_t* h_chr_is_autosome, int32_t counts_per_bin, int32_t bin_size_in,
                                     int32_t* d_chr, int32_t* d_start, int32_t* d_stop, int32_t* d_gc, float* d_count, int64_t cap,
                                     int32_t* h_bin_size_out, int64_t* h_nbins_per_chr, int64_t* h_nbins_total);
int32_t canvas_bin_gcw_stats(canvas_ctx* ctx, int64_t* h_out2);

int32_t canvas_bin_predefined(canvas_ctx* ctx, int32_t nchr, const uint8_t* const* d_bases, const uint64_t* const* d_mask, const uint8_t* const* d_hits, const int64_t* h_len,
                              int32_t mode, const int64_t* h_bin_offset, const int32_t* h_bin_start, const int32_t* h_bin_stop, const int32_t* d_bin_start, const int32_t* d_bin_stop,
                              int32_t* d_gc, float* d_count);
int32_t canvas_bin_predefined_gcweighted(canvas_ctx* ctx, int32_t nchr, const uint8_t* const* d_bases, const uint64_t* const* d_mask, const uint8_t* const* d_hits,
                                         const int16_t* const* d_fraglen, const int64_t* h_len, const int64_t* h_bin_offset, const int32_t* h_bin_start, const int32_t* h_bin_stop,
                                         const int32_t* d_bin_start, const int32_t* d_bin_stop, int32_t* d_gc, float* d_count);

int32_t canvas_clean(canvas_ctx* ctx, int64_t n, int32_t* d_chr, int32_t* d_start, int32_t* d_stop, float* d_count,
                     int32_t* d_gc, int32_t nchr, const uint8_t* h_chr_is_autosome, uint32_t flags, int32_t min_bins_per_gc,
                     double* h_local_sd_out, int64_t* h_n_out, int32_t* h_info);

int32_t canvas_clean2(canvas_ctx* ctx, int64_t n, int32_t* d_chr, int32_t* d_start, int32_t* d_stop, float* d_count,
                      int32_t* d_gc, int32_t nchr, const uint8_t* h_chr_is_autosome, const uint8_t* h_chr_is_y, uint32_t flags,
                      int32_t min_bins_per_gc, double* h_local_sd_out, int64_t* h_n_out, int32_t* h_info);
int32_t canvas_clean_batch(canvas_ctx* ctx, int32_t nsamples, const int64_t* h_n, int32_t* const* h_d_chr, int32_t* const* h_d_start, int32_t* const* h_d_stop, float* const* h_d_count,
                           int32_t* const* h_d_gc, int32_t nchr, const uint8_t* h_chr_is_autosome, const uint8_t* h_chr_is_y, uint32_t flags, int32_t min_bins_per_gc,
                           double* h_local_sd_out, int64_t* h_n_out, int32_t* h_info);
int32_t canvas_merge_cleaned(canvas_ctx* ctx, int32_t nsamples, const int64_t* h_n, const int32_t* const* h_d_chr, const int32_t* const* h_d_start,
                             const int32_t* const* h_d_stop, const float* const* h_d_count, int32_t* d_out_chr, int32_t* d_out_start, int32_t* d_out_stop,
                             float* const* h_d_out_count, int64_t* h_n_out);
int32_t canvas_chromosome_offsets(canvas_ctx* ctx, const int32_t* d_chr, int64_t n, int32_t nchr, int64_t* h_chr_offset);

int32_t canvas_quantize_f2(canvas_ctx* ctx, const float* d_count, int64_t n, double* d_cov);

int32_t canvas_hmm_per_sample(canvas_ctx* ctx, int32_t nchr, const double* d_cov, const int64_t* h_chr_offset, int32_t* d_state);
int32_t canvas_hmm_joint(canvas_ctx* ctx, int32_t nsamples, int32_t nchr, const double* const* h_d_cov, const int64_t* h_chr_offset, int32_t* d_state);
int32_t canvas_segment_ids(canvas_ctx* ctx, int32_t nchr, const int64_t* h_chr_offset, const int32_t* d_state,
                           const int32_t* d_start, const int32_t* d_stop, int32_t max_inter_bin_dist, int32_t* d_segment_id,
                           int64_t* h_nsegments);
int32_t canvas_segment_ids_filtered(canvas_ctx* ctx, int32_t nchr, const int64_t* h_chr_offset, const int32_t* d_state,
                                    const int32_t* d_start, const int32_t* d_stop, int32_t max_inter_bin_dist,
                                    const int64_t* h_excl_offset, const int32_t* h_excl_start, const int32_t* h_excl_stop,
                                    int32_t* d_segment_id, int64_t* h_nsegments);
int32_t canvas_segment_ids_ploidy(canvas_ctx* ctx, int32_t nchr, const int64_t* h_chr_offset, const int32_t* d_state, const int32_t* d_start,
                                  const int32_t* d_stop, int32_t max_inter_bin_dist,
                                  const int64_t* h_excl_offset, const int32_t* h_excl_start, const int32_t* h_excl_stop,
                                  const int64_t* h_ploidy_offset, const int32_t* h_ploidy_start, const int32_t* h_ploidy_end, const int32_t* h_ploidy_cn,
                                  int32_t* d_segment_id, int64_t* h_nsegments);
int32_t canvas_evenness_score(canvas_ctx* ctx, int32_t nchr, const double* d_cov, const int64_t* h_chr_offset, int32_t window_size, double* h_score, int32_t* h_valid);
int32_t canvas_split_overlapping(int32_t nsamples, const uint32_t* const* h_start, const uint32_t* const* h_end, const int32_t* h_nseg,
                                 uint32_t* h_out_start, uint32_t* h_out_end, int32_t cap, int32_t* h_nout);
int32_t canvas_cbs(canvas_ctx* ctx, int32_t nchr, const double* d_cov, const int64_t* h_chr_offset, double alpha, uint32_t nperm,
                   int32_t* d_seg_len, int32_t* h_nseg, int64_t* h_stats);

int32_t canvas_cbs_undo(canvas_ctx* ctx, int32_t nchr, const double* d_cov, const int64_t* h_chr_offset, double alpha, uint32_t nperm,
                        int32_t undo, double undo_sd, int32_t* d_seg_len, int32_t* h_nseg, int64_t* h_stats);

int32_t canvas_cbs_device_stats(canvas_ctx* ctx, int64_t* h_out6);
int32_t canvas_cbs_tpermp_stats(canvas_ctx* ctx, int64_t* h_out2);
int32_t canvas_cbs_tailp_stats(canvas_ctx* ctx, int64_t* h_out2);
int32_t canvas_cbs_tail_probe(canvas_ctx* ctx, const double* h_x, int32_t n, double tol, double* h_nu, int32_t* h_flag);
int32_t canvas_cbs_perm_probe(canvas_ctx* ctx, const double* h_x, int32_t n, uint32_t seed, int32_t nb, int32_t kernel, double tss, double* h_lohi, double* h_ms3);
int32_t canvas_cbs_arc_probe(canvas_ctx* ctx, int32_t mode, int32_t nseg, const int64_t* h_off, const double* h_x, int32_t al0, int32_t pair_cap,
                             double* h_sx, double* h_tau, double* h_stat, int32_t* h_iseg, int32_t* h_path, uint64_t* h_words, double* h_dmax, int32_t* h_first);
int32_t canvas_select_probe(canvas_ctx* ctx, int32_t variant, int32_t dtype, const void* d_values, int32_t nseg, const int64_t* h_seg_off, int32_t nq,
                            const int32_t* h_seg_lo, const int32_t* h_seg_hi, const int64_t* h_k, uint64_t* h_keys_out);
int32_t canvas_hmm_backbone_probe(canvas_ctx* ctx, int32_t mode, int32_t nchr, const int64_t* h_chr_offset, const double* d_V, double* d_carry, int32_t* h_fail);
int64_t canvas_cbs_boundary(uint32_t nperm, double alpha, uint32_t* h_out, int64_t cap);
int32_t canvas_cbs_prefetch(canvas_ctx* ctx, int32_t nchr, int64_t words_per_chromosome);
int32_t canvas_cbs_stream_read(canvas_ctx* ctx, int32_t chromosome, int64_t position, int64_t nwords, uint32_t* h_out);
int32_t canvas_cbs_cache_stats(canvas_ctx* ctx, int64_t* h_out6);
int32_t canvas_cbs_seeds(int32_t nchr, int32_t* h_out, int32_t* h_variant);

int32_t canvas_wavelets(canvas_ctx* ctx, int32_t nchr, const double* d_cov, const int64_t* h_chr_offset, int32_t is_germline,
                        double threshold_lower, double threshold_upper, double mad_factor, int32_t variability_window, int32_t min_size,
                        int32_t* h_breakpoints, int64_t cap, int64_t* h_bp_offset);
int32_t canvas_wavelets_stats(canvas_ctx* ctx, int64_t* h_out2);
int32_t canvas_wavelets_decisions(canvas_ctx* ctx, int64_t* h_out4);
int32_t canvas_wavelets_inputs(canvas_ctx* ctx, int32_t nchr, int32_t* h_has_cv, double* h_cv, double* h_f3_9, uint8_t* h_is_root, double* h_median, double* h_sigma, double* h_keep_above,
                               int32_t* h_paths);
int32_t canvas_wavelets_prefix_probe(canvas_ctx* ctx, int32_t nchr, const double* d_cov, const int64_t* h_chr_offset, int64_t* h_p1, int64_t* h_p2, int32_t* h_bad2);
int32_t canvas_wavelets_bound_probe(canvas_ctx* ctx, int32_t nchr, const double* d_cov, const int64_t* h_chr_offset, int32_t nnodes, const int32_t* h_nodes3, double* h_t, double* h_b);
int32_t canvas_wavelets_level_probe(canvas_ctx* ctx, int32_t nchr, const double* d_cov, const int64_t* h_chr_offset, int32_t nnodes, const int32_t* h_nodes4, const double* h_keep_above,
                                    int32_t wv_long, int32_t* h_status, int32_t* h_ind, int32_t* h_next4, int64_t* h_nnext, int32_t* h_roots6, int64_t* h_nroots, int32_t* h_counts,
                                    int32_t* h_overflow);
int32_t canvas_wavelets_chain_probe(canvas_ctx* ctx, int64_t n_cov, const double* d_cov, int32_t nnodes, const int32_t* h_nodes2, const int32_t* h_lim, int32_t fast, int32_t own_slices,
                                    double* h_coef, int32_t* h_ind, int32_t* h_flag);
int32_t canvas_wavelets_subtree_probe(canvas_ctx* ctx, int32_t nchr, const double* d_cov, const int64_t* h_chr_offset, int32_t nroots, const int32_t* h_roots6, const double* h_keep_above,
                                      int64_t cap_cand, int32_t wv_long, int32_t use_table, int32_t* h_counts, int32_t* h_cand5, double* h_cand_coef, int64_t* h_ncand, int32_t* h_overflow);
int32_t canvas_wavelets_median_probe(canvas_ctx* ctx, int64_t n_cov, const double* d_cov, int32_t nstretch, const int64_t* h_start, const int64_t* h_len, double* h_median, double* h_median_wg,
                                     int32_t* h_bad2);

int32_t canvas_sample_pipeline(canvas_ctx* ctx, int32_t nchr, const uint8_t* const* d_bases, const uint64_t* const* d_mask, const uint8_t* const* d_hits,
                               const int64_t* h_len, const uint8_t* h_chr_is_autosome, const uint8_t* h_chr_is_y, int32_t counts_per_bin, int32_t bin_size_in,
                               int32_t mode, uint32_t clean_flags, int32_t min_bins_per_gc, int32_t max_inter_bin_dist,
                               int32_t* d_chr, int32_t* d_start, int32_t* d_stop, int32_t* d_gc, float* d_count, int64_t cap,
                               double* d_cov, int32_t* d_state, int32_t* d_segment_id,
                               int32_t* h_bin_size, int64_t* h_nbins, int64_t* h_nbins_clean, double* h_local_sd, int64_t* h_chr_offset, int64_t* h_nsegments);

int32_t canvas_sample_pipeline_packed(canvas_ctx* ctx, int32_t nchr, const uint64_t* const* d_ref, const uint64_t* const* d_hit_planes, const int64_t* h_len, const int64_t* h_pos0,
                                      const uint8_t* h_chr_is_autosome, const uint8_t* h_chr_is_y, int32_t counts_per_bin, int32_t bin_size_in,
                                      int32_t mode, uint32_t clean_flags, int32_t min_bins_per_gc, int32_t max_inter_bin_dist,
                                      int32_t* d_chr, int32_t* d_start, int32_t* d_stop, int32_t* d_gc, float* d_count, int64_t cap,
                                      double* d_cov, int32_t* d_state, int32_t* d_segment_id,
                                      int32_t* h_bin_size, int64_t* h_nbins, int64_t* h_nbins_clean, double* h_local_sd, int64_t* h_chr_offset, int64_t* h_nsegments);

int32_t canvas_normalize_reference(canvas_ctx* ctx, int32_t nsamples, const double* const* h_d_counts, int64_t n, const int32_t* d_on_target_idx, int64_t n_on_target,
                                   double* d_weighted, double* h_weights);
int32_t canvas_normalize_ratio(canvas_ctx* ctx, int64_t n, const float* d_sample, const float* d_reference, const int32_t* d_on_target_idx, int64_t n_on_target,
                               int32_t mode, double min_ref, double max_ref, const int32_t* d_ploidy, int32_t* d_keep_idx, float* d_ratio, float* d_count,
                               int64_t* h_n_out, double* h_library_size_factor);
int32_t canvas_normalize_best_normal(canvas_ctx* ctx, const double* d_tumor, int32_t nnormals, const double* const* h_d_normals, int64_t n, const int32_t* d_on_target_idx,
                                     int64_t n_on_target, int32_t* h_best, double* h_mean_sq_log_ratio, int64_t* h_ignored, int32_t* h_replayed);
int32_t canvas_normalize_pca_reference(canvas_ctx* ctx, int64_t n, const float* d_sample, const float* d_mu, int32_t naxes, const double* const* h_d_axes,
                                       double min_ref, double max_ref, float* d_reference, double* h_median_ratio, double* h_sizes, int32_t* h_orthogonal);

int32_t canvas_comm_unique_id(void* h_id128);
int32_t canvas_comm_init(canvas_ctx* ctx, int32_t rank, int32_t nranks, const void* h_id128);
typedef int32_t (*canvas_host_allgather_fn)(void* user, const void* send, int64_t bytes_per_rank, void* recv);
int32_t canvas_comm_init_host(canvas_ctx* ctx, int32_t rank, int32_t nranks, canvas_host_allgather_fn fn, void* user);
int32_t canvas_comm_split(canvas_ctx* ctx, int32_t color, int32_t key);
int32_t canvas_comm_restore(canvas_ctx* ctx);
int32_t canvas_comm_rank(canvas_ctx* ctx, int32_t* h_rank, int32_t* h_nranks);
int32_t canvas_allgather_boundaries(canvas_ctx* ctx, const int32_t* d_local, int32_t nlocal, int32_t max_per_rank,
                                    int32_t* d_all, int32_t* h_counts);

int32_t canvas_bin_sample_sharded(canvas_ctx* ctx, int32_t nchr, const int32_t* h_chr_owner, const uint8_t* const* d_bases, const uint64_t* const* d_mask,
                                  const uint8_t* const* d_hits, const int16_t* const* d_fraglen, const int64_t* h_len, const uint8_t* h_chr_is_autosome,
                                  int32_t counts_per_bin, int32_t bin_size_in, int32_t mode, int32_t* d_chr, int32_t* d_start, int32_t* d_stop, int32_t* d_gc, float* d_count,
                                  int64_t cap, int32_t* h_bin_size, int64_t* h_nbins);
int32_t canvas_sample_pipeline_sharded(canvas_ctx* ctx, int32_t nchr, const int32_t* h_chr_owner, const uint8_t* const* d_bases, const uint64_t* const* d_mask,
                                       const uint8_t* const* d_hits, const int64_t* h_len, const uint8_t* h_chr_is_autosome, const uint8_t* h_chr_is_y,
                                       int32_t counts_per_bin, int32_t bin_size_in, int32_t mode, uint32_t clean_flags, int32_t min_bins_per_gc, int32_t max_inter_bin_dist,
                                       int32_t* d_chr, int32_t* d_start, int32_t* d_stop, int32_t* d_gc, float* d_count, int64_t cap,
                                       double* d_cov, int32_t* d_state, int32_t* d_segment_id,
                                       int32_t* h_bin_size, int64_t* h_nbins, int64_t* h_nbins_clean, double* h_local_sd, int64_t* h_chr_offset, int64_t* h_nsegments);
int32_t canvas_sample_pipeline_sharded_packed(canvas_ctx* ctx, int32_t nchr, const int32_t* h_chr_owner, const uint64_t* const* d_ref, const uint64_t* const* d_hit_planes,
                                              const int64_t* h_len, const int64_t* h_pos0, const uint8_t* h_chr_is_autosome, const uint8_t* h_chr_is_y,
                                              int32_t counts_per_bin, int32_t bin_size_in, int32_t mode, uint32_t clean_flags, int32_t min_bins_per_gc, int32_t max_inter_bin_dist,
                                              int32_t* d_chr, int32_t* d_start, int32_t* d_stop, int32_t* d_gc, float* d_count, int64_t cap,
                                              double* d_cov, int32_t* d_state, int32_t* d_segment_id,
                                              int32_t* h_bin_size, int64_t* h_nbins, int64_t* h_nbins_clean, double* h_local_sd, int64_t* h_chr_offset, int64_t* h_nsegments);
int32_t canvas_sharded_stats(canvas_ctx* ctx, int64_t* h_out6);
int32_t canvas_cbs_sharded(canvas_ctx* ctx, int32_t nchr, const int32_t* h_chr_owner, const double* d_cov, const int64_t* h_chr_offset, double alpha, uint32_t nperm,
                           int32_t undo, double undo_sd, int32_t* d_seg_len, int32_t* h_nseg, int64_t* h_stats);
int32_t canvas_hmm_per_sample_sharded(canvas_ctx* ctx, int32_t nchr, const int32_t* h_chr_owner, const double* d_cov, const int64_t* h_chr_offset, int32_t* d_state);
int32_t canvas_wavelets_sharded(canvas_ctx* ctx, int32_t nchr, const int32_t* h_chr_owner, const double* d_cov, const int64_t* h_chr_offset, int32_t is_germline,
                                double threshold_lower, double threshold_upper, double mad_factor, int32_t variability_window, int32_t min_size,
                                int32_t* h_breakpoints, int64_t cap, int64_t* h_bp_offset);

// ... 171 lines not shown
```

Before: 1.924 billion bins/s.

## Fuse segment-id flagging into Viterbi backtrack and run the id scan inside the backbone walk

Backtracking now computes the per-bin increments and segment-start flags in the same pass that writes states, and counts flags per 2048-bin block with ballots and atomics. The separate flag, count and scan kernels are replaced by extra waves appended to the backbone walk launch, which scan block counts and write segment ids. Pair maps are composed on the fly instead of being materialised, and the block counters are zeroed in the setup kernel. This cuts several launches and global passes over the state array. In exchange the walk kernel carries a mixed role and depends on atomic counters and launch ordering being correct.

```diff
diff --git a/canvas_amd/csrc/hmm.hip b/canvas_amd/csrc/hmm.hip
--- a/canvas_amd/csrc/hmm.hip
+++ b/canvas_amd/csrc/hmm.hip
@@ -366,7 +366,8 @@
 template <typename VB_T, typename BB_T>
 __global__ void __launch_bounds__(256) k_hmm_setup(const HmmDescPack pack, int usePack, HmmDescDev D, int nchr,
                                                    int nblocks, int nblocksS, int nchunks, int vb, int vbs, int bbChunk, VB_T* __restrict__ vBlocks, VB_T* __restrict__ sBlocks, BB_T* __restrict__ bChunks,
-                                                   const double* __restrict__ cov, int64_t N, double maxThreshold, int32_t* __restrict__ idx, int32_t* __restrict__ dLast, int32_t* __restrict__ dFail) {
+                                                   const double* __restrict__ cov, int64_t N, double maxThreshold, int32_t* __restrict__ idx, int32_t* __restrict__ dLast, int32_t* __restrict__ dFail,
+                                                   uint32_t* __restrict__ segCnt, int nbSeg) {
     const int32_t* first = usePack ? pack.first : D.first; const int32_t* firstS = usePack ? pack.firstS : D.firstS; const int32_t* firstChunk = usePack ? pack.firstChunk : D.firstChunk;
     if (usePack && blockIdx.x == 0) {
         for (int c = threadIdx.x; c < nchr; c += 256) D.chroms[c] = pack.chroms[c];
@@ -377,6 +378,7 @@
     if (i < nblocksS) make_block_entry(firstS, nchr, (int)i, vbs, sBlocks);
     if (i < nchunks) make_block_entry(firstChunk, nchr, (int)i, bbChunk, bChunks);
     if (i < nchr) { dLast[i] = -1; dFail[i] = 0; }
+    if (segCnt && i < nbSeg) segCnt[i] = 0u;
     if (cov && i < N) {
         double x = cov[i];
         x = x > maxThreshold ? maxThreshold : x;
@@ -465,20 +467,20 @@
     return lo;
 }
 #define VBS (VB / 2)
-__global__ void __launch_bounds__(256) k_pair_maps(const VitBlock* __restrict__ blocks, int nblocks, const HmmChrom* __restrict__ chroms, const int32_t* __restrict__ firstS,
-                                                   const uint16_t* __restrict__ mapsS, uint16_t* __restrict__ maps, const int32_t* __restrict__ todo) {
-    const int b = blockIdx.x * 256 + threadIdx.x;
-    if (b >= nblocks) return;
-    const VitBlock B = blocks[b];
-    if (todo && !todo[B.chrom]) return;
-    const int64_t T = chroms[B.chrom].T;
-    const int s0 = firstS[B.chrom] + B.t0 / VBS;
+__device__ __forceinline__ uint32_t vit_pair_map(const uint16_t* __restrict__ mapsS, int firstS, int64_t t0, int64_t T) {
+    const int s0 = firstS + (int)(t0 / VBS);
     uint32_t m = mapsS[s0];
 #pragma unroll
-    for (int k = 1; k < VB / VBS; k++) if (B.t0 + (int64_t)k * VBS < T) m = map_compose(m, mapsS[s0 + k]);
-    maps[b] = (uint16_t)m;
-}
-
+    for (int k = 1; k < VB / VBS; k++) if (t0 + (int64_t)k * VBS < T) m = map_compose(m, mapsS[s0 + k]);
+    return m;
+}
+
+__device__ __forceinline__ double vit_increment(const HmmParams& P, const double* __restrict__ logPmf, int s1, int sPrev, int ix, bool first) {
+    if (s1 < 0) return 0.0;
+    const double e = logPmf[(size_t)s1 * P.tableLen + ix];
+    if (first) { const double lik = e + P.logA[0][s1]; return P.logPi[s1] + lik - P.logA[0][s1]; }
+    return e + P.logA[sPrev < 0 ? 0 : sPrev][s1];
+}
 __global__ void __launch_bounds__(256) k_vit_increments(const HmmChrom* __restrict__ chroms, int nchr, const int64_t* __restrict__ chrOff, const int32_t* __restrict__ idx,
                                                         const double* __restrict__ logPmf, HmmParams P, const int32_t* __restrict__ state, int64_t N, double* __restrict__ D) {
     __shared__ int64_t sOff[CHR_LDS_CAP];
@@ -488,10 +490,7 @@
     const int s1 = state[g], sPrev = state[g > 0 ? g - 1 : 0], ix = idx[g];
     const int lo = chrom_of_bin(off, nchr, g);
     const int64_t begin = chroms[lo].begin;
-    if (s1 < 0) { D[g] = 0.0; return; }
-    double e = logPmf[(size_t)s1 * P.tableLen + ix];
-    if (g == begin) { double lik = e + P.logA[0][s1]; D[g] = P.logPi[s1] + lik - P.logA[0][s1]; }
-    else { const int s0 = sPrev; D[g] = e + P.logA[s0 < 0 ? 0 : s0][s1]; }
+    D[g] = vit_increment(P, logPmf, s1, sPrev, ix, g == begin);
 }
 
 __global__ void __launch_bounds__(64) k_vit_backbone(const HmmChrom* __restrict__ chroms, const double* __restrict__ V, double* __restrict__ carryOut, const int32_t* __restrict__ todo = nullptr) {
@@ -776,8 +775,40 @@
     bits = ((unsigned long long)e << 52) | (k2 & MANT);
     return true;
 }
+struct SegIdRole { int nwalk = 0; int nb = 0; const uint8_t* flags = nullptr; const uint32_t* blockCnt = nullptr; int64_t n = 0; int32_t* segId = nullptr;
+                   unsigned long long* total = nullptr; unsigned* totalSeq = nullptr; unsigned seq = 0; };
+__device__ __forceinline__ void seg_ids_wave(const SegIdRole& R, int blk) {
+    const int l = threadIdx.x;
+    const int64_t base = (int64_t)blk * 2048;
+    uint32_t w[8];
+#pragma unroll
+    for (int q = 0; q < 8; q++) { const int64_t i = base + q * 256 + 4 * l; w[q] = i < R.n ? *reinterpret_cast<const uint32_t*>(R.flags + i) : 0u; }
+    uint32_t mine = 0;
+    for (int j = l; j < blk; j += 64) mine += R.blockCnt[j];
+    uint32_t running = wave_reduce_add_u32(mine);
+#pragma unroll
+    for (int q = 0; q < 8; q++) {
+        const int64_t i = base + q * 256 + 4 * l;
+        uint32_t f[4], sum = 0;
+#pragma unroll
+        for (int k = 0; k < 4; k++) { f[k] = (i + k < R.n) ? ((w[q] >> (8 * k)) & 1u) : 0u; sum += f[k]; }
+        const uint32_t inc = wave_inclusive_scan_u32(sum);
+        uint32_t id = running + inc - sum;
+        VecI4 out;
+#pragma unroll
+        for (int k = 0; k < 4; k++) { id += f[k]; out.v[k] = (int32_t)id - 1; }
+        if (i + 3 < R.n) *reinterpret_cast<VecI4*>(R.segId + i) = out;
+        else {
+#pragma unroll
+            for (int k = 0; k < 4; k++) if (i + k < R.n) R.segId[i + k] = out.v[k];
+        }
+        running += (uint32_t)__builtin_amdgcn_readlane((int)inc, 63);
+    }
+    if (blk == R.nb - 1 && l == 0) { *R.total = running; cvx_mail_publish(R.totalSeq, R.seq); }
+}
 __global__ void __launch_bounds__(64) k_bb_walk(const int32_t* __restrict__ firstChunk, const BbChunkOut* __restrict__ chunkOut, const BbCross* __restrict__ cross,
-                                                unsigned long long* __restrict__ chunkBits, BbPost* __restrict__ post, int32_t* __restrict__ fail) {
+                                                unsigned long long* __restrict__ chunkBits, BbPost* __restrict__ post, int32_t* __restrict__ fail, const SegIdRole R) {
+    if (R.nb > 0 && (int)blockIdx.x >= R.nwalk) { seg_ids_wave(R, (int)blockIdx.x - R.nwalk); return; }
     __shared__ BbCross sCr[BB_MAXC];
     const int c = blockIdx.x, l = threadIdx.x;
     const unsigned long long MANT = (1ull << 52) - 1ull;
@@ -1011,6 +1042,7 @@
     maps[b] = (uint16_t)m;
 }
 __global__ void __launch_bounds__(64) k_bt_group(const int32_t* __restrict__ firstBlock, const int32_t* __restrict__ firstGroup, int nchr, const uint16_t* __restrict__ maps,
+                                                 const HmmChrom* __restrict__ chroms, const int32_t* __restrict__ firstS, const uint16_t* __restrict__ mapsS,
                                                  uint16_t* __restrict__ pre, uint16_t* __restrict__ gmap) {
     const int g = blockIdx.x, l = threadIdx.x;
     int lo = 0, hi = nchr - 1;
@@ -1018,7 +1050,8 @@
     while (lo < nchr - 1 && firstGroup[lo + 1] <= g) lo++;
     const int first = firstBlock[lo], last = firstBlock[lo + 1] - 1;
     const int bi = last - ((g - firstGroup[lo]) * 64 + l);
-    uint32_t f = bi >= first ? (uint32_t)maps[bi] : MAP_IDENT;
+    uint32_t f = MAP_IDENT;
+    if (bi >= first) f = mapsS ? vit_pair_map(mapsS, firstS[lo], (int64_t)(bi - first) * VB, chroms[lo].T) : (uint32_t)maps[bi];
 #pragma unroll
     for (int dlt = 1; dlt < 64; dlt <<= 1) { const uint32_t o = __shfl_up(f, dlt); if (l >= dlt) f = map_compose(f, o); }
     const uint32_t ex = __shfl_up(f, 1);
@@ -1064,6 +1097,80 @@
     const uint32_t m0 = map_compose(a0, ex), m1 = map_compose(x1, ex);
     if (j0 < cnt) state[C.begin + tEnd - 1 - j0] = s < 0 ? s : (int)map_get(m0, (uint32_t)s);
     if (j1 < cnt) state[C.begin + tEnd - 1 - j1] = s < 0 ? s : (int)map_get(m1, (uint32_t)s);
+}
+struct SegFlagOut { const int32_t* start; const int32_t* stop; int32_t maxDist; uint8_t* flags; uint32_t* blockCnt; };
+__device__ __forceinline__ bool seg_flag_plain(int st, int stPrev, bool first, int32_t stopPrev, int32_t startHere, int32_t maxDist) {
+    bool newSeg = st >= 0 && (first || stPrev != st);
+    if (!newSeg && !first) {
+        const uint32_t prevEnd = (uint32_t)stopPrev;
+        if (prevEnd > 0 && maxDist >= 0 && (uint64_t)prevEnd + (uint64_t)maxDist < (uint64_t)(uint32_t)startHere) newSeg = true;
+    }
+    return newSeg;
+}
+template <bool SEG>
+__global__ void __launch_bounds__(256) k_bt_states_inc(const VitBlock* __restrict__ blocks, int nblocks, const HmmChrom* __restrict__ chroms, const uint16_t* __restrict__ psi,
+                                                       const int32_t* __restrict__ firstBlock, const int32_t* __restrict__ firstGroup, const int32_t* __restrict__ firstS,
+                                                       const uint16_t* __restrict__ mapsS, const uint16_t* __restrict__ pre, const int8_t* __restrict__ gentry,
+                                                       const int32_t* __restrict__ idx, const double* __restrict__ logPmf, HmmParams P,
+                                                       int32_t* __restrict__ state, double* __restrict__ D, SegFlagOut G) {
+    static_assert(VB <= 128, "two steps per lane");
+    const int b = blockIdx.x * 4 + (threadIdx.x >> 6), l = lane_id();
+    if (b >= nblocks) return;
+    const VitBlock B = blocks[b];
+    const HmmChrom C = chroms[B.chrom];
+    const int64_t tBeg = B.t0, tEnd = (B.t0 + VB < C.T) ? B.t0 + VB : C.T;
+    const int cnt = (int)(tEnd - tBeg);
+    const int sg = gentry[firstGroup[B.chrom] + (firstBlock[B.chrom + 1] - 1 - b) / 64];
+    const int s = sg < 0 ? sg : (int)map_get((uint32_t)pre[b], (uint32_t)sg);
+    const uint32_t mb = vit_pair_map(mapsS, firstS[B.chrom], tBeg, C.T);
+    const int sBefore = s < 0 ? s : (int)map_get(mb, (uint32_t)s);
+    const int j0 = 2 * l, j1 = 2 * l + 1;
+    const bool on0 = j0 < cnt, on1 = j1 < cnt;
+    const int64_t g0 = C.begin + tEnd - 1 - j0, g1 = g0 - 1;
+    const bool first0 = tEnd - 1 - j0 == 0, first1 = tEnd - 1 - j1 == 0;
+    const uint32_t a0 = (j0 >= 1 && on0) ? (uint32_t)psi[C.begin + tEnd - j0] : MAP_IDENT;
+    const uint32_t a1 = on1 ? (uint32_t)psi[C.begin + tEnd - j1] : MAP_IDENT;
+    const int ix0 = on0 ? idx[g0] : 0, ix1 = on1 ? idx[g1] : 0;
+    int32_t start0 = 0, start1 = 0, stopP0 = 0, stopP1 = 0;
+    if (SEG) {
+        if (on0) start0 = G.start[g0];
+        if (on1) start1 = G.start[g1];
+        if (on0 && !first0) stopP0 = G.stop[g0 - 1];
+        if (on1 && !first1) stopP1 = G.stop[g1 - 1];
+    }
+    const uint32_t x1 = map_compose(a1, a0);
+    uint32_t v = x1;
+#pragma unroll
+    for (int d = 1; d < 64; d <<= 1) { const uint32_t o = __shfl_up(v, d); if (l >= d) v = map_compose(v, o); }
+    uint32_t ex = __shfl_up(v, 1);
+    if (l == 0) ex = MAP_IDENT;
+    const uint32_t m0 = map_compose(a0, ex), m1 = map_compose(x1, ex);
+    const int st0 = s < 0 ? s : (int)map_get(m0, (uint32_t)s), st1 = s < 0 ? s : (int)map_get(m1, (uint32_t)s);
+    const int stNext = __shfl_down(st0, 1);
+    const int sp0 = on1 ? st1 : sBefore;
+    const int sp1 = j1 + 1 < cnt ? stNext : sBefore;
+    if (on0) { state[g0] = st0; D[g0] = vit_increment(P, logPmf, st0, sp0, ix0, first0); }
+    if (on1) { state[g1] = st1; D[g1] = vit_increment(P, logPmf, st1, sp1, ix1, first1); }
+    if (SEG) {
+        const bool f0 = on0 && seg_flag_plain(st0, sp0, first0, stopP0, start0, G.maxDist);
+        const bool f1 = on1 && seg_flag_plain(st1, sp1, first1, stopP1, start1, G.maxDist);
+        if (on0) G.flags[g0] = f0;
+        if (on1) G.flags[g1] = f1;
+        const int64_t blkLo = (C.begin + tBeg) >> 11;
+        const bool hi0 = (g0 >> 11) != blkLo, hi1 = (g1 >> 11) != blkLo;
+        const uint32_t cLo = (uint32_t)(__popcll(__ballot(f0 && !hi0)) + __popcll(__ballot(f1 && !hi1)));
+        const uint32_t cHi = (uint32_t)(__popcll(__ballot(f0 && hi0)) + __popcll(__ballot(f1 && hi1)));
+        if (l == 0) { if (cLo) atomicAdd(&G.blockCnt[blkLo], cLo); if (cHi) atomicAdd(&G.blockCnt[blkLo + 1], cHi); }
+    }
+}
+__global__ void __launch_bounds__(64) k_seg_flags_short(const HmmChrom* __restrict__ chroms, SegFlagOut G) {
+    const HmmChrom C = chroms[blockIdx.x];
+    const int l = threadIdx.x;
+    if (C.T > 10 || l >= C.T) return;
+    const int64_t g = C.begin + l;
+    const bool f = seg_flag_plain(-1, -1, l == 0, l > 0 ? G.stop[g - 1] : 0, G.start[g], G.maxDist);
+    G.flags[g] = f;
+    if (f) atomicAdd(&G.blockCnt[g >> 11], 1u);
 }
 
 __global__ void __launch_bounds__(256) k_fill_i32(int32_t* __restrict__ p, int64_t begin, int64_t end, int32_t v) {
@@ -1371,14 +1478,16 @@
     return W;
 }
 static void enqueue_backbone(canvas_ctx* ctx, int mode, int nchr, int nchunks, const HmmChrom* dChroms, const BbChunk* dBChunks, const int32_t* dFirstChunk, const double* dV,
-                             double* dCarry, int32_t* dFail, const int32_t* dTodo, const BbWork& W) {
+                             double* dCarry, int32_t* dFail, const int32_t* dTodo, const BbWork& W, const SegIdRole* segRole = nullptr ) {
     if (mode == BB_MODE_CHAIN) hipLaunchKernelGGL(k_vit_backbone, dim3(nchr), dim3(64), 0, ctx->stream, dChroms, dV, dCarry, dTodo);
     else if (mode == BB_MODE_SCAN) hipLaunchKernelGGL(k_vit_backbone_scan, dim3(nchr), dim3(BS_T), 0, ctx->stream, dChroms, dV, dCarry, dFail);
     else {
         hipLaunchKernelGGL(k_bb_sums, dim3(nchunks), dim3(256), 0, ctx->stream, dBChunks, dChroms, dV, W.chunkSum, dFail);
         hipLaunchKernelGGL(k_bb_bases, dim3(nchr), dim3(64), 0, ctx->stream, dFirstChunk, W.chunkSum, W.chunkBase);
         hipLaunchKernelGGL(k_bb_pieces, dim3(nchunks), dim3(256), 0, ctx->stream, dBChunks, dChroms, dV, W.chunkBase, W.chunkOut, W.cross, W.at64Fn, W.at64Rank, dFail);
-        hipLaunchKernelGGL(k_bb_walk, dim3(nchr), dim3(64), 0, ctx->stream, dFirstChunk, W.chunkOut, W.cross, W.chunkBits, W.post, dFail);
+        SegIdRole R; if (segRole) R = *segRole;
+        R.nwalk = nchr;
+        hipLaunchKernelGGL(k_bb_walk, dim3(nchr + R.nb), dim3(64), 0, ctx->stream, dFirstChunk, W.chunkOut, W.cross, W.chunkBits, W.post, dFail, R);
         hipLaunchKernelGGL(k_bb_emit, dim3(nblk2((int64_t)nchunks * 16, 256)), dim3(256), 0, ctx->stream, dBChunks, nchunks, dChroms, W.chunkBits, W.post, W.at64Fn, W.at64Rank, dCarry);
     }
 }
@@ -1416,8 +1525,6 @@
 struct HmmEmis { int32_t* idx = nullptr; double* dTab = nullptr;
                  const double* indexCov = nullptr; };
 struct SegPost { const int32_t* d_start; const int32_t* d_stop; int32_t maxDist; int32_t* d_segment_id; int64_t nseg = 0; bool valid = false; };
-static void enqueue_segment_ids(canvas_ctx* ctx, const int64_t* dOff, int nchr, const int32_t* d_state, const int32_t* d_start, const int32_t* d_stop, int64_t N, int32_t maxDist,
-                                uint8_t* flags, uint32_t* blockCnt, unsigned long long* dTot, int32_t* d_segment_id, unsigned* totSeq = nullptr, unsigned seq = 0);
 template <class PrepareA, class PrepareB>
 static int32_t hmm_pipeline(canvas_ctx* ctx, int32_t nchr, const int64_t* h_chr_offset, size_t extraBytes, PrepareA prepareA, PrepareB prepareB, int32_t* d_state, SegPost* seg = nullptr,
                             bool descByValue = false ) {
@@ -1480,10 +1587,10 @@
     ctx->hmm_dispersion = 1e9;
     rc = prepareA(ws, P, E, (const HmmChrom*)dChroms, (const int64_t*)dOffDev); if (rc) return rc;
     {
-        const int64_t most = std::max<int64_t>(std::max<int64_t>(E.indexCov ? N : 0, nblocks), std::max<int64_t>(std::max(nblocksS, nchunks), nchr));
+        const int64_t most = std::max<int64_t>(std::max<int64_t>(E.indexCov ? N : 0, std::max(nblocks, seg ? nbSeg : 0)), std::max<int64_t>(std::max(nblocksS, nchunks), nchr));
         HmmDescDev DD{dChroms, dOffDev, dFirst, dFirstChunk, dFirstS, dFirstGroup};
         hipLaunchKernelGGL((k_hmm_setup<VitBlock, BbChunk>), dim3(nblk2(most, 256)), dim3(256), 0, ctx->stream, pack, byVal ? 1 : 0, DD, nchr, nblocks, nblocksS, nchunks, VB, VBS, BB_CHUNK,
-                           dVBlocks, dSBlocks, dBChunks, E.indexCov, N, P.maxThreshold, E.idx, dLast, dFail);
+                           dVBlocks, dSBlocks, dBChunks, E.indexCov, N, P.maxThreshold, E.idx, dLast, dFail, segBlockCnt, nbSeg);
     }
     rc = prepareB(ws, P, E); if (rc) return rc;
     int32_t* idx = E.idx; double* dTab = E.dTab;
@@ -1493,14 +1600,19 @@
         if (chroms[c].T <= 10 && chroms[c].T > 0)
             hipLaunchKernelGGL(k_fill_i32, dim3(nblk2(chroms[c].T, 256)), dim3(256), 0, ctx->stream, d_state, chroms[c].begin, chroms[c].begin + chroms[c].T, -1);
     const unsigned laneGrid = (unsigned)((nblocks + 63) / 64);
-    auto backtrack = [&](bool haveMaps) {
+    auto backtrack = [&](bool specMaps, const SegFlagOut* segOut) {
         if (nblocks > 0) {
-            if (!haveMaps) hipLaunchKernelGGL(k_bt_maps, dim3(nblk2(nblocks, 256)), dim3(256), 0, ctx->stream, dVBlocks, nblocks, dChroms, psi, dMaps);
-            hipLaunchKernelGGL(k_bt_group, dim3(ngroups), dim3(64), 0, ctx->stream, dFirst, dFirstGroup, nchr, dMaps, dPre, dGmap);
+            if (!specMaps) hipLaunchKernelGGL(k_bt_maps, dim3(nblk2(nblocks, 256)), dim3(256), 0, ctx->stream, dVBlocks, nblocks, dChroms, psi, dMaps);
+            hipLaunchKernelGGL(k_bt_group, dim3(ngroups), dim3(64), 0, ctx->stream, dFirst, dFirstGroup, nchr, dMaps, dChroms, dFirstS, specMaps ? dMapsS : (const uint16_t*)nullptr, dPre, dGmap);
             hipLaunchKernelGGL(k_bt_gchain, dim3(nchr), dim3(64), 0, ctx->stream, dFirstGroup, dLast, dGmap, dGentry);
-            hipLaunchKernelGGL(k_bt_states, dim3(nblk2(nblocks, 4)), dim3(256), 0, ctx->stream, dVBlocks, nblocks, dChroms, psi, dFirst, dFirstGroup, dPre, dGentry, d_state);
+            const dim3 gb(nblk2(nblocks, 4));
+            if (!specMaps) hipLaunchKernelGGL(k_bt_states, gb, dim3(256), 0, ctx->stream, dVBlocks, nblocks, dChroms, psi, dFirst, dFirstGroup, dPre, dGentry, d_state);
+            else if (segOut) hipLaunchKernelGGL((k_bt_states_inc<true>), gb, dim3(256), 0, ctx->stream, dVBlocks, nblocks, dChroms, psi, dFirst, dFirstGroup, dFirstS, dMapsS, dPre, dGentry, idx, dTab, P, d_state, dD, *segOut);
+            else hipLaunchKernelGGL((k_bt_states_inc<false>), gb, dim3(256), 0, ctx->stream, dVBlocks, nblocks, dChroms, psi, dFirst, dFirstGroup, dFirstS, dMapsS, dPre, dGentry, idx, dTab, P, d_state, dD, SegFlagOut{});
         }
     };
+    bool anyShort = false;
+    for (int c = 0; c < nchr; c++) anyShort = anyShort || (chroms[c].T > 0 && chroms[c].T <= 10);
     bool twoValuedAll = true;
     for (int i = 0; i < NSTATE; i++) for (int j = 0; j < NSTATE; j++) {
         const double ref = i == j ? P.logA[0][0] : P.logA[0][1];
@@ -1528,20 +1640,32 @@
             else if (lds) hipLaunchKernelGGL((k_vit_spec<true, false>), gs, dim3(64), lds, ctx->stream, dSBlocks, nblocksS, dChroms, idx, dTab, P, psi, dMapsS, dLast, leadSpec, dTodo, VBS);
             else if (twoValued) hipLaunchKernelGGL((k_vit_spec<false, true>), gs, dim3(64), 0, ctx->stream, dSBlocks, nblocksS, dChroms, idx, dTab, P, psi, dMapsS, dLast, leadSpec, dTodo, VBS);
             else hipLaunchKernelGGL((k_vit_spec<false, false>), gs, dim3(64), 0, ctx->stream, dSBlocks, nblocksS, dChroms, idx, dTab, P, psi, dMapsS, dLast, leadSpec, dTodo, VBS);
-            hipLaunchKernelGGL(k_pair_maps, dim3(nblk2(nblocks, 256)), dim3(256), 0, ctx->stream, dVBlocks, nblocks, dChroms, dFirstS, dMapsS, dMaps, dTodo);
             if (attempt < corrupt.attempts) hipLaunchKernelGGL(k_vit_corrupt, dim3(1), dim3(64), 0, ctx->stream, psi, chroms[corrupt.chrom].begin + corrupt.t, corrupt.state);
-            backtrack(true);
-            hipLaunchKernelGGL(k_vit_increments, dim3(nblk2(N, 256)), dim3(256), 0, ctx->stream, dChroms, nchr, dOffDev, idx, dTab, P, d_state, N, dD);
+            const bool segNow = seg && attempt == 0 && (!corrupt.on || corrupt.retry);
+            SegFlagOut segOut{};
+            if (segNow) {
+                segOut = SegFlagOut{seg->d_start, seg->d_stop, seg->maxDist, segFlags, segBlockCnt};
+                if (anyShort) hipLaunchKernelGGL(k_seg_flags_short, dim3(nchr), dim3(64), 0, ctx->stream, dChroms, segOut);
+            }
+            backtrack(true, segNow ? &segOut : nullptr);
             const char* bbMode = cvx_hook("CANVAS_HMM_BACKBONE");
             const int bb = ((bbMode && !strcmp(bbMode, "chain")) || (attempt > 1 && !bbMode)) ? BB_MODE_CHAIN : ((bbMode && !strcmp(bbMode, "scan")) ? BB_MODE_SCAN : BB_MODE_PIECES);
-            enqueue_backbone(ctx, bb, nchr, nchunks, dChroms, dBChunks, dFirstChunk, dD, dCarry, dFail, dTodo, bbWork);
+            SegIdRole segRole;
+            if (segNow) {
+                (void)segTot;
+                segSeq = cvx_mail_arm(ctx, hSegSeq);
+                segRole.nb = nbSeg; segRole.flags = segFlags; segRole.blockCnt = segBlockCnt; segRole.n = N; segRole.segId = seg->d_segment_id;
+                segRole.total = hSegTot ; segRole.totalSeq = hSegSeq; segRole.seq = segSeq;
+            }
+            enqueue_backbone(ctx, bb, nchr, nchunks, dChroms, dBChunks, dFirstChunk, dD, dCarry, dFail, dTodo, bbWork, segNow && bb == BB_MODE_PIECES ? &segRole : nullptr);
             if (lds) hipLaunchKernelGGL((k_vit_verify<true>), dim3(laneGrid), dim3(64), lds, ctx->stream, dVBlocks, nblocks, dChroms, idx, dTab, P, psi, d_state, dD, dCarry, dLast, dFail, leadVer, dTodo);
             else hipLaunchKernelGGL((k_vit_verify<false>), dim3(laneGrid), dim3(64), 0, ctx->stream, dVBlocks, nblocks, dChroms, idx, dTab, P, psi, d_state, dD, dCarry, dLast, dFail, leadVer, dTodo);
             CANVAS_HIP_TRY(ctx, hipMemcpyAsync(hFail, dFail, nchr * 4, hipMemcpyDeviceToHost, ctx->stream));
-            if (seg && attempt == 0 && (!corrupt.on || corrupt.retry)) {
-                (void)segTot;
-                segSeq = cvx_mail_arm(ctx, hSegSeq);
-                enqueue_segment_ids(ctx, dOffDev, nchr, d_state, seg->d_start, seg->d_stop, N, seg->maxDist, segFlags, segBlockCnt, hSegTot , seg->d_segment_id, hSegSeq, segSeq);
+            if (segNow) {
+                if (bb != BB_MODE_PIECES) {
+                    hipLaunchKernelGGL(k_scan_blocks2, dim3(1), dim3(1024), 0, ctx->stream, segBlockCnt, nbSeg, hSegTot, hSegSeq, segSeq);
+                    hipLaunchKernelGGL(k_seg_ids, dim3(nbSeg), dim3(256), 0, ctx->stream, segFlags, segBlockCnt, N, seg->d_segment_id);
+                }
                 segEnqueued = true;
             }
             CANVAS_HIP_TRY(ctx, hipStreamSynchronize(ctx->stream));
@@ -1565,7 +1689,7 @@
         if (cvx_hook("CANVAS_HMM_DEBUG_FAIL")) { fprintf(stderr, "viterbi sequential kernel for %zu chromosomes (speculative %d, blocks %d):", redo.size(), (int)speculative, nblocks); for (size_t i = 0; i < redo.size() && i < 6; i++) fprintf(stderr, " chr%d(T=%lld)", redo[i], (long long)chroms[redo[i]].T); fprintf(stderr, "\n"); }
         rc = canvas_h2d_small(ctx, dRedo, redo.data(), redo.size() * 4); if (rc) return rc;
         hipLaunchKernelGGL(k_viterbi, dim3((unsigned)redo.size()), dim3(64), lds, ctx->stream, dChroms, idx, dTab, P, psi, dLast, dRedo);
-        backtrack(false);
+        backtrack(false, nullptr);
     }
     ctx->hmm_redo = (int)redo.size();
     CANVAS_HIP_TRY(ctx, hipStreamSynchronize(ctx->stream));
@@ -1849,15 +1973,16 @@
     return CANVAS_OK;
 }
 
-static void enqueue_segment_ids(canvas_ctx* ctx, const int64_t* dOff, int nchr, const int32_t* d_state, const int32_t* d_start, const int32_t* d_stop, int64_t N, int32_t maxDist,
-                                uint8_t* flags, uint32_t* blockCnt, unsigned long long* dTot, int32_t* d_segment_id, unsigned* totSeq, unsigned seq) {
-    const int nb = (int)nblk2(N, 2048);
-    hipLaunchKernelGGL(k_seg_flags, dim3(nblk2(N, 256)), dim3(256), 0, ctx->stream, dOff, nchr, d_state, d_start, d_stop, N, maxDist, (const int64_t*)nullptr, (const int32_t*)nullptr, (const int32_t*)nullptr,
-                       (const int64_t*)nullptr, (const int32_t*)nullptr, (const int32_t*)nullptr, (const int32_t*)nullptr, flags);
-    hipLaunchKernelGGL(k_count_blocks, dim3(nb), dim3(256), 0, ctx->stream, flags, N, blockCnt);
-    hipLaunchKernelGGL(k_scan_blocks2, dim3(1), dim3(1024), 0, ctx->stream, blockCnt, nb, dTot, totSeq, seq);
-    hipLaunchKernelGGL(k_seg_ids, dim3(nb), dim3(256), 0, ctx->stream, flags, blockCnt, N, d_segment_id);
-}
+extern "C" int32_t canvas_hmm_segments_probe(canvas_ctx* ctx, int32_t nchr, const double* d_cov, const int64_t* h_chr_offset, const int32_t* d_start, const int32_t* d_stop,
+                                             int32_t max_inter_bin_dist, int32_t* d_state, int32_t* d_segment_id, int64_t* h_nsegments) {
+    if (!ctx) return CANVAS_ERR_INVALID;
+    if (nchr < 1 || nchr > (1 << 20) || !h_chr_offset || !h_nsegments) CANVAS_FAIL(ctx, CANVAS_ERR_INVALID, "canvas_hmm_segments_probe: bad arguments (1..2^20 chromosomes)");
+    if (h_chr_offset[0] != 0) CANVAS_FAIL(ctx, CANVAS_ERR_INVALID, "canvas_hmm_segments_probe: the offsets start at 0");
+    for (int c = 0; c < nchr; c++) if (h_chr_offset[c + 1] < h_chr_offset[c] || h_chr_offset[c + 1] > (1ll << 30)) CANVAS_FAIL(ctx, CANVAS_ERR_INVALID, "canvas_hmm_segments_probe: the offsets decrease or pass 2^30 bins");
+    if (!d_cov || !d_start || !d_stop || !d_state || !d_segment_id) CANVAS_FAIL(ctx, CANVAS_ERR_INVALID, "canvas_hmm_segments_probe: missing arrays");
+    return cvx_hmm_per_sample_segments(ctx, nchr, d_cov, h_chr_offset, d_state, nullptr , d_start, d_stop, max_inter_bin_dist, d_segment_id, h_nsegments);
+}
+
 extern "C" {
 int32_t canvas_segment_ids_ploidy(canvas_ctx* ctx, int32_t nchr, const int64_t* h_chr_offset, const int32_t* d_state, const int32_t* d_start,
                                   const int32_t* d_stop, int32_t max_inter_bin_dist, const int64_t* h_excl_offset, const int32_t* h_excl_start,
diff --git a/canvas_amd/lib.py b/canvas_amd/lib.py
--- a/canvas_amd/lib.py
+++ b/canvas_amd/lib.py
@@ -21,7 +21,7 @@
     "canvas_mask_from_fasta", "canvas_mask_exclude_intervals", "canvas_screen_hits",
     "canvas_bin_rates", "canvas_bin_size_from_rates", "canvas_bin_count_upper_bound", "canvas_bin_genome", "canvas_bin_sample", "canvas_bin_sample_gcweighted", "canvas_bin_predefined", "canvas_bin_predefined_gcweighted",
     "canvas_clean", "canvas_clean2", "canvas_clean_batch", "canvas_merge_cleaned", "canvas_chromosome_offsets", "canvas_quantize_f2", "canvas_hmm_per_sample", "canvas_hmm_joint", "canvas_segment_ids", "canvas_segment_ids_filtered", "canvas_segment_ids_ploidy", "canvas_evenness_score", "canvas_split_overlapping", "canvas_cbs", "canvas_cbs_undo", "canvas_cbs_device_stats", "canvas_cbs_tailp_stats", "canvas_cbs_tail_probe", "canvas_cbs_boundary", "canvas_cbs_seeds", "canvas_cbs_prefetch", "canvas_cbs_stream_read", "canvas_cbs_cache_stats", "canvas_wavelets", "canvas_wavelets_stats", "canvas_wavelets_decisions", "canvas_wavelets_inputs", "canvas_wavelets_prefix_probe", "canvas_wavelets_bound_probe", "canvas_wavelets_level_probe", "canvas_wavelets_chain_probe", "canvas_wavelets_subtree_probe", "canvas_wavelets_median_probe", "canvas_normalize_reference", "canvas_normalize_ratio", "canvas_normalize_best_normal", "canvas_normalize_pca_reference", "canvas_sample_pipeline",
-    "canvas_comm_unique_id", "canvas_comm_init", "canvas_comm_init_host", "canvas_allgather_boundaries", "canvas_sample_pipeline_sharded", "canvas_sample_pipeline_sharded_packed", "canvas_sharded_stats", "canvas_cbs_sharded", "canvas_wavelets_sharded", "canvas_allgather_host", "canvas_merge_cleaned_sharded", "canvas_profile_enable", "canvas_profile_get", "canvas_bin_gcw_stats", "canvas_cbs_tpermp_stats", "canvas_comm_split", "canvas_comm_restore", "canvas_comm_rank", "canvas_bin_sample_sharded", "canvas_hmm_per_sample_sharded", "canvas_cbs_perm_probe", "canvas_cbs_arc_probe", "canvas_stale_reads", "canvas_select_probe", "canvas_hmm_backbone_probe",
+    "canvas_comm_unique_id", "canvas_comm_init", "canvas_comm_init_host", "canvas_allgather_boundaries", "canvas_sample_pipeline_sharded", "canvas_sample_pipeline_sharded_packed", "canvas_sharded_stats", "canvas_cbs_sharded", "canvas_wavelets_sharded", "canvas_allgather_host", "canvas_merge_cleaned_sharded", "canvas_profile_enable", "canvas_profile_get", "canvas_bin_gcw_stats", "canvas_cbs_tpermp_stats", "canvas_comm_split", "canvas_comm_restore", "canvas_comm_rank", "canvas_bin_sample_sharded", "canvas_hmm_per_sample_sharded", "canvas_cbs_perm_probe", "canvas_cbs_arc_probe", "canvas_stale_reads", "canvas_select_probe", "canvas_hmm_backbone_probe", "canvas_hmm_segments_probe",
     "canvas_memcpy_h2d_async", "canvas_snv_count", "canvas_flag_unique_kmers", "canvas_fasta_case_from_mask",
     "canvas_smooth", "canvas_smooth_lengths", "canvas_smooth_plan",
     "canvas_segment_select", "canvas_segment_select_plan", "canvas_call_diploid",
@@ -570,6 +570,19 @@
         fail = np.zeros(len(off) - 1, np.int32)
         self._check(self.lib.canvas_hmm_backbone_probe(self.ctx, C.c_int32(mode), C.c_int32(len(off) - 1), _np_ptr(off), C.c_void_p(dv.data_ptr()), C.c_void_p(dc.data_ptr()), _np_ptr(fail)))
         return dc.cpu().numpy()[:n].view(np.float64), fail
+
+    def hmm_segments_probe(self, cov, chr_offset, start, stop, max_inter_bin_dist=1000000):
+        torch = self.torch
+        off = np.ascontiguousarray(chr_offset, np.int64)
+        n = int(off[-1])
+        if cov.dtype != torch.float64 or start.dtype != torch.int32 or stop.dtype != torch.int32 or min(cov.numel(), start.numel(), stop.numel()) < n:
+            raise CanvasError("hmm_segments_probe: float64 coverage and int32 start / stop of chr_offset[-1] elements")
+        state = torch.empty(max(n, 1), dtype=torch.int32, device=self.device); seg = torch.empty(max(n, 1), dtype=torch.int32, device=self.device)
+        torch.cuda.synchronize(self.device)
+        nseg = C.c_int64(0)
+        self._check(self.lib.canvas_hmm_segments_probe(self.ctx, C.c_int32(len(off) - 1), C.c_void_p(cov.data_ptr()), _np_ptr(off), C.c_void_p(start.data_ptr()), C.c_void_p(stop.data_ptr()),
+                                                       C.c_int32(max_inter_bin_dist), C.c_void_p(state.data_ptr()), C.c_void_p(seg.data_ptr()), C.byref(nseg)))
+        return state[:n], seg[:n], nseg.value
 
     def stale_reads(self):
         out = np.zeros(2, np.int64)
diff --git a/include/canvas_hip.h b/include/canvas_hip.h
--- a/include/canvas_hip.h
+++ b/include/canvas_hip.h
@@ -138,6 +138,8 @@
 int32_t canvas_select_probe(canvas_ctx* ctx, int32_t variant, int32_t dtype, const void* d_values, int32_t nseg, const int64_t* h_seg_off, int32_t nq,
                             const int32_t* h_seg_lo, const int32_t* h_seg_hi, const int64_t* h_k, uint64_t* h_keys_out);
 int32_t canvas_hmm_backbone_probe(canvas_ctx* ctx, int32_t mode, int32_t nchr, const int64_t* h_chr_offset, const double* d_V, double* d_carry, int32_t* h_fail);
+int32_t canvas_hmm_segments_probe(canvas_ctx* ctx, int32_t nchr, const double* d_cov, const int64_t* h_chr_offset, const int32_t* d_start, const int32_t* d_stop,
+                                  int32_t max_inter_bin_dist, int32_t* d_state, int32_t* d_segment_id, int64_t* h_nsegments);
 int64_t canvas_cbs_boundary(uint32_t nperm, double alpha, uint32_t* h_out, int64_t cap);
 int32_t canvas_cbs_prefetch(canvas_ctx* ctx, int32_t nchr, int64_t words_per_chromosome);
 int32_t canvas_cbs_stream_read(canvas_ctx* ctx, int32_t chromosome, int64_t position, int64_t nwords, uint32_t* h_out);
```

After: 1.963 billion bins/s, median of 6. 2.0% higher.
